# mhalushka/miRge3.0

Measured on AMD Instinct MI355X. Metric: M reads/s through full annotation cascade; per-class counts bit-exact vs ref, higher is better.
Workload: dtype u64

## Files before the change

mirge3.0_amd/csrc/kernels_join.hpp:

```cpp
#pragma once
#define MIRGE_JOIN_LDS 2048
__global__ void k_join(const int8_t* __restrict__ res_pass, const int32_t* __restrict__ res_ref,
                       const uint32_t* __restrict__ counts, uint32_t n, int32_t S, int32_t n_pass,
                       int32_t exact_pass, int32_t iso_pass, unsigned long long* __restrict__ class_sums,
                       unsigned long long* __restrict__ exact, unsigned long long* __restrict__ iso) {
    __shared__ unsigned long long acc[MIRGE_JOIN_LDS];
    const int cells = n_pass * S;
    const bool use_lds = cells <= MIRGE_JOIN_LDS;
    if (use_lds) {
        for (int c = threadIdx.x; c < cells; c += blockDim.x) acc[c] = 0ull;
        __syncthreads();
    }
    for (uint32_t i = blockIdx.x * blockDim.x + threadIdx.x; i < n; i += gridDim.x * blockDim.x) {
        const int p = res_pass[i];
        if (p < 0) continue;
        const int32_t ref = res_ref[i];
        for (int32_t s = 0; s < S; s++) {
            const unsigned long long c = counts[(size_t)i * S + s];
            if (!c) continue;
            if (use_lds) atomicAdd(&acc[p * S + s], c);
            else atomicAdd(&class_sums[p * S + s], c);
            if (p == exact_pass) atomicAdd(&exact[(size_t)ref * S + s], c);
            else if (p == iso_pass) atomicAdd(&iso[(size_t)ref * S + s], c);
        }
    }
    if (use_lds) {
        __syncthreads();
        for (int c = threadIdx.x; c < cells; c += blockDim.x)
            if (acc[c]) atomicAdd(&class_sums[c], acc[c]);
    }
}

struct JoinGroups {
    const int8_t* pass[MIRGE_NCLS];
    const int32_t* ref[MIRGE_NCLS];
    const uint32_t* counts[MIRGE_NCLS];
    uint32_t start[MIRGE_NCLS + 1];
    int32_t n_groups;
};
__global__ void k_join_multi(JoinGroups gs, int32_t S, int32_t n_pass, int32_t exact_pass, int32_t iso_pass,
                             unsigned long long* __restrict__ class_sums, unsigned long long* __restrict__ exact,
                             unsigned long long* __restrict__ iso) {
    __shared__ unsigned long long acc[MIRGE_JOIN_LDS];
    const int cells = n_pass * S;
    const bool use_lds = cells <= MIRGE_JOIN_LDS;
    if (use_lds) {
        for (int c = threadIdx.x; c < cells; c += blockDim.x) acc[c] = 0ull;
        __syncthreads();
    }
    const uint32_t total = gs.start[gs.n_groups];
    for (uint32_t t = blockIdx.x * blockDim.x + threadIdx.x; t < total; t += gridDim.x * blockDim.x) {
        int k = 0;
#pragma unroll
        for (int q = 1; q < MIRGE_NCLS; q++) if (q < gs.n_groups && t >= gs.start[q]) k = q;
        const uint32_t i = t - gs.start[k];
        const int8_t* gp = nullptr; const int32_t* gr = nullptr; const uint32_t* gc = nullptr;
#pragma unroll
        for (int q = 0; q < MIRGE_NCLS; q++) if (q == k) { gp = gs.pass[q]; gr = gs.ref[q]; gc = gs.counts[q]; }
        const int p = gp[i];
        if (p < 0) continue;
        const int32_t ref = gr[i];
        for (int32_t s = 0; s < S; s++) {
            const unsigned long long c = gc[(size_t)i * S + s];
            if (!c) continue;
            if (use_lds) atomicAdd(&acc[p * S + s], c);
            else atomicAdd(&class_sums[p * S + s], c);
            if (p == exact_pass) atomicAdd(&exact[(size_t)ref * S + s], c);
            else if (p == iso_pass) atomicAdd(&iso[(size_t)ref * S + s], c);
        }
    }
    if (use_lds) {
        __syncthreads();
        for (int c = threadIdx.x; c < cells; c += blockDim.x)
            if (acc[c]) atomicAdd(&class_sums[c], acc[c]);
    }
}

#define MIRGE_JOIN_ROWS_THREADS 1024
#define MIRGE_JOIN_ROWS_CELLS 6144
__global__ void __launch_bounds__(MIRGE_JOIN_ROWS_THREADS)
k_join_rows(JoinGroups gs, int32_t S, int32_t n_pass, int32_t exact_pass, int32_t iso_pass, uint32_t n_tab,
            unsigned long long* __restrict__ partial) {
    extern __shared__ __attribute__((aligned(16))) unsigned long long j_acc[];
    const uint32_t n_cls = (uint32_t)(n_pass * S), W = n_cls + 2 * n_tab;
    for (uint32_t c = threadIdx.x; c < W; c += blockDim.x) j_acc[c] = 0ull;
    __syncthreads();
    const uint32_t total = gs.start[gs.n_groups];
    if (gs.n_groups == 1 && S == 1) {
        const int8_t* __restrict__ gp = gs.pass[0]; const int32_t* __restrict__ gr = gs.ref[0]; const uint32_t* __restrict__ gc = gs.counts[0];
        const uint64_t stride = (uint64_t)gridDim.x * blockDim.x;
        for (uint64_t t0 = (uint64_t)blockIdx.x * blockDim.x + threadIdx.x; t0 < total; t0 += 4 * stride) {
            int p[4]; uint32_t r[4]; unsigned long long c[4];
#pragma unroll
            for (int u = 0; u < 4; u++) {
                const uint64_t i = t0 + (uint64_t)u * stride;
                const bool in = i < total;
                p[u] = in ? (int)gp[i] : -1;
                r[u] = in ? (uint32_t)gr[i] : 0u;
                c[u] = in ? (unsigned long long)gc[i] : 0ull;
            }
#pragma unroll
            for (int u = 0; u < 4; u++) {
                if (p[u] < 0 || !c[u]) continue;
                atomicAdd(&j_acc[p[u]], c[u]);
                if (p[u] == exact_pass) atomicAdd(&j_acc[n_cls + r[u]], c[u]);
                else if (p[u] == iso_pass) atomicAdd(&j_acc[n_cls + n_tab + r[u]], c[u]);
            }
        }
    } else
    for (uint32_t t = blockIdx.x * blockDim.x + threadIdx.x; t < total; t += gridDim.x * blockDim.x) {
        int k = 0;
#pragma unroll
        for (int q = 1; q < MIRGE_NCLS; q++) if (q < gs.n_groups && t >= gs.start[q]) k = q;
        const int8_t* gp = gs.pass[0]; const int32_t* gr = gs.ref[0]; const uint32_t* gc = gs.counts[0];
#pragma unroll
        for (int q = 1; q < MIRGE_NCLS; q++) if (q == k) { gp = gs.pass[q]; gr = gs.ref[q]; gc = gs.counts[q]; }
        const uint32_t i = t - gs.start[k];
        const int p = gp[i];
        if (p < 0) continue;
        const uint32_t ref = (uint32_t)gr[i];
        for (int32_t s = 0; s < S; s++) {
            const unsigned long long c = gc[(size_t)i * S + s];
            if (!c) continue;
            atomicAdd(&j_acc[p * S + s], c);
            if (p == exact_pass) atomicAdd(&j_acc[n_cls + (size_t)ref * S + s], c);
            else if (p == iso_pass) atomicAdd(&j_acc[n_cls + n_tab + (size_t)ref * S + s], c);
        }
    }
    __syncthreads();
    unsigned long long* row = partial + (size_t)blockIdx.x * W;
    for (uint32_t c = threadIdx.x; c < W; c += blockDim.x) row[c] = j_acc[c];
}
__global__ void __launch_bounds__(1024)
k_join_reduce(const unsigned long long* __restrict__ partial, uint32_t rows, uint32_t W, unsigned long long* __restrict__ tables,
              unsigned long long* __restrict__ host_out) {
    __shared__ unsigned long long s_part[16][64];
    const uint32_t lane = threadIdx.x & 63, wave = threadIdx.x >> 6;
    const uint32_t c = blockIdx.x * 64 + lane;
    unsigned long long sum = 0ull;
    if (c < W)
        for (uint32_t r = wave; r < rows; r += 16) sum += partial[(size_t)r * W + c];
    s_part[wave][lane] = sum;
    __syncthreads();
    if (wave == 0 && c < W) {
        unsigned long long tot = 0ull;
#pragma unroll
        for (int w = 0; w < 16; w++) tot += s_part[w][lane];
        if (host_out) host_out[c] = tables[c] + tot;
        else if (tot) tables[c] += tot;
    }
}

template <typename T>
__global__ void k_scatter_out(const T* __restrict__ in, uint32_t n, uint32_t base,
                              const uint32_t* __restrict__ orig, T* __restrict__ out) {
    for (uint32_t j = blockIdx.x * blockDim.x + threadIdx.x; j < n; j += gridDim.x * blockDim.x)
        out[orig ? orig[j] : base + j] = in[j];
}



#define MIRGE_TALLY_MAXPOS 32
struct TallyOut {
    unsigned long long *n_seqs, *seq_true, *count_true, *canon, *kept_exact, *census;
    int8_t *diag, *state;
};

struct TallyMember {
    const int8_t* res_pass; const int32_t* res_ref; const uint32_t* counts; int32_t S, exact_pass, iso_pass;
    const int32_t* fam_of_ref; const double* freq;
    __device__ __forceinline__ bool operator()(uint32_t i) const {
        const int p = res_pass[i];
        if (p != exact_pass && p != iso_pass) return false;
        const int32_t f = fam_of_ref[res_ref[i]];
        bool member = f >= 0 && p == exact_pass;
        if (f >= 0 && p == iso_pass)
            for (int32_t s = 0; s < S; s++) member |= (double)counts[(size_t)i * S + s] * freq[s] >= 1.0;
        return member;
    }
};
struct IsoMember {
    const int8_t* res_pass; int32_t exact_pass, iso_pass; const uint32_t* orig; uint32_t base; const int32_t* slot_of_read;
    __device__ __forceinline__ bool operator()(uint32_t i) const {
        const int p = res_pass[i];
        return (p == exact_pass || p == iso_pass) && slot_of_read[orig ? orig[i] : base + i] >= 0;
    }
};

template <class Pred, int BLOCK>
__global__ void k_member_list(uint32_t n, uint32_t chunk, Pred pred, uint32_t* __restrict__ list, uint32_t* __restrict__ n_list) {
    __shared__ uint32_t s_wave[BLOCK / 64 + 1];
    const int lane = threadIdx.x & 63, wave = threadIdx.x >> 6;
    const uint32_t lo = blockIdx.x * chunk, hi = min(n, lo + chunk);
    uint32_t run = 0;
    for (uint32_t i0 = lo; i0 < hi; i0 += BLOCK) {
        const uint32_t i = i0 + threadIdx.x;
        const bool member = i < hi && pred(i);
        const unsigned long long bal = __ballot(member);
        if (lane == 0) s_wave[wave] = (uint32_t)__popcll(bal);
        __syncthreads();
        uint32_t before = 0, tot = 0;
#pragma unroll
        for (int w = 0; w < BLOCK / 64; w++) { const uint32_t c = s_wave[w]; if (w < wave) before += c; tot += c; }
        if (member) list[lo + run + before + (uint32_t)__popcll(bal & ((1ull << lane) - 1ull))] = i;
        run += tot;
        __syncthreads();
    }
    if (threadIdx.x == 0) n_list[blockIdx.x] = run;
}

__global__ void k_tally(GroupView<1> g, uint32_t base, const uint32_t* __restrict__ orig, const int8_t* __restrict__ res_pass,
                        const int32_t* __restrict__ res_ref, const uint32_t* __restrict__ counts, int32_t S,
                        int32_t exact_pass, int32_t iso_pass, const int32_t* __restrict__ fam_of_ref,
                        const uint64_t* __restrict__ tgt_bits, const uint8_t* __restrict__ tgt_len,
                        const uint8_t* __restrict__ retained, const double* __restrict__ freq, TallyOut o,
                        const uint32_t* __restrict__ list, const uint32_t* __restrict__ n_list, uint32_t chunk) {
    const uint32_t n_members = n_list[blockIdx.x];
    for (uint32_t k = threadIdx.x; k < n_members; k += blockDim.x) {
        const uint32_t i = list[(size_t)blockIdx.x * chunk + k];
        const int p = res_pass[i];
        const uint32_t h = orig ? orig[i] : base + i;
        const int32_t f = fam_of_ref[res_ref[i]];
        const uint64_t tw = tgt_bits[f];
        const int Lt = tgt_len[f], Lr = g.len[i];
        const uint64_t rw = g.seq[i];
        const uint64_t rn = g.nmask ? g.nmask[i] : 0ull;
        int best = 0, best_i = 0, best_j = 0, d = 0;
        const int nd = Lr + Lt - 1;
        for (int k = 0; k < nd + 3; k++) {
            const int dd = k < 3 ? k - 1 : k - 3 - (Lr - 1);
            if (dd <= -Lr || dd >= Lt) continue;
            const int i0 = dd > 0 ? dd : 0, i1 = min(Lt, dd + Lr), j0 = i0 - dd;
            if (2 * (i1 - i0) < best) continue;
            const uint64_t x = (tw >> (2 * i0)) ^ (rw >> (2 * j0));
            uint64_t m2 = ((x | (x >> 1)) & 0x5555555555555555ull) | ((rn >> (2 * j0)) & 0x5555555555555555ull);
            m2 = (m2 | (m2 >> 1)) & 0x3333333333333333ull;
            m2 = (m2 | (m2 >> 2)) & 0x0F0F0F0F0F0F0F0Full;
            m2 = (m2 | (m2 >> 4)) & 0x00FF00FF00FF00FFull;
            m2 = (m2 | (m2 >> 8)) & 0x0000FFFF0000FFFFull;
            const uint32_t mis = (uint32_t)(m2 | (m2 >> 16));
            int run = 0;
            for (int t = 0; t < i1 - i0; t++) {
                run = max(0, run + (((mis >> t) & 1u) ? -1 : 2));
                const int ti = i0 + t, rj = j0 + t;
                if (run > best || (run == best && run > 0 && (ti < best_i || (ti == best_i && rj < best_j)))) {
                    best = run; best_i = ti; best_j = rj; d = dd;
                }
            }
        }
        bool state = d <= 1;
        if (state) {
            const int hd_t = d < 0 ? -d : 0, hd_s = d > 0 ? d : 0;
            const int A = max(hd_t + Lt, hd_s + Lr);
            const int last = min(A - hd_t - 1 - 3, hd_s + Lr - 1);
            int mism = 0, match = 0;
            for (int pos = hd_t; pos <= last; pos++) {
                const int rj = pos - hd_s, q = pos - hd_t;
                if (rj < 0) continue;
                const bool eq = q < Lt && !((rn >> (2 * rj)) & 1ull) && (((tw >> (2 * q)) & 3ull) == ((rw >> (2 * rj)) & 3ull));
                if (eq) match++; else mism++;
            }
            state = !(mism > 1 || match < Lt - 3 - 1 - (d == 1 ? 1 : 0));
        }
        o.diag[h] = (int8_t)d;
        o.state[h] = state ? 1 : 0;
        const bool keep = state && (!retained || retained[h]);
        bool sub = false;
        if (keep && rn == 0ull && Lr <= Lt) {
            const uint64_t m = mirge_lowmask2(Lr);
            for (int a = 0; a + Lr <= Lt && !sub; a++) sub = ((tw >> (2 * a)) & m) == rw;
        }
        for (int32_t s = 0; s < S; s++) {
            const unsigned long long c = counts[(size_t)i * S + s];
            if (!c) continue;
            const size_t fs = (size_t)f * S + s;
            atomicAdd(&o.n_seqs[fs], 1ull);
            if (keep) {
                atomicAdd(&o.seq_true[fs], 1ull);
                atomicAdd(&o.count_true[fs], c);
                if (sub) atomicAdd(&o.canon[fs], c);
                if (p == exact_pass) atomicAdd(&o.kept_exact[fs], 1ull);
            }
            for (int q = max(0, d); q < Lt - 5 && q - d < Lr; q++) {
                const int rj = q - d;
                if ((rn >> (2 * rj)) & 1ull) continue;
                const int cb = (int)((tw >> (2 * q)) & 3ull), rb = (int)((rw >> (2 * rj)) & 3ull);
                if (cb == rb) continue;
                unsigned long long* cell = &o.census[((((size_t)f * MIRGE_TALLY_MAXPOS + q) * 16 + cb * 4 + rb) * 3) * S + s];
                atomicAdd(cell, c);
                if (state) atomicAdd(cell + S, c);
                if (keep) atomicAdd(cell + 2 * S, c);
            }
        }
    }
}
```

mirge3.0_amd/csrc/native_cascade.hpp:

```cpp
#pragma once
struct ResGroup {
    uint32_t n = 0;
    int8_t* pass = nullptr;
    uint32_t* pos = nullptr;
    int8_t* mm = nullptr;
    int32_t* ref = nullptr;
    int32_t* off = nullptr;
};
struct mirge_result {
    mirge_ctx* ctx = nullptr;
    int64_t n = 0;
    int32_t n_pass = 0;
    ResGroup g[MIRGE_NGROUPS];
    const mirge_reads* reads = nullptr;
    uint32_t n_refs[MIRGE_MAX_PASSES] = {0};
    uint32_t* dmeta = nullptr;
};

extern "C" void mirge_result_destroy(mirge_result* r) {
    if (!r) return;
    (void)join_pending_now(r->ctx);
    for (auto& g : r->g) {
        r->ctx->release(g.pass); r->ctx->release(g.pos); r->ctx->release(g.mm);
        r->ctx->release(g.ref); r->ctx->release(g.off);
    }
    r->ctx->release(r->dmeta);
    delete r;
}

static int merged_library(mirge_ctx* c, const mirge_lib* const* members, int n, mirge_lib** out) {
    std::vector<uint64_t> uids;
    for (int i = 0; i < n; i++) uids.push_back(members[i]->uid);
    for (auto& m : c->merged)
        if (m.uids == uids) { *out = m.lib; return 0; }
    std::string seq;
    std::vector<int64_t> off;
    std::vector<const MirgeHostLib*> hl;
    for (int i = 0; i < n; i++) hl.push_back(&members[i]->h);
    merged_library_text(hl.data(), n, seq, off);
    mirge_lib* L = nullptr;
    CHECK(mirge_lib_create(c, seq.data(), off.data(), (int64_t)off.size() - 1, &L));
    c->merged.push_back(mirge_ctx::Merged{uids, L});
    *out = L;
    return 0;
}

static int prepare_tables(mirge_lib* lib, const mirge_policy& pol, const int32_t* hist, bool long_present) {
    MirgePolicy p;
    std::memcpy(&p, &pol, sizeof(p));
    std::vector<ShapeJob> wanted;
    std::vector<bool> seen(MIRGE_SHAPE_SLOTS, false);
    for (int L = 1; L <= MIRGE_MAX_READ_LEN + 1; L++) {
        const bool lng = L > MIRGE_MAX_READ_LEN;
        if (lng ? !long_present : !hist[L]) continue;
        if (p.len_lt > 0 && !(L < p.len_lt) && !(lng && p.len_lt > MIRGE_MAX_READ_LEN + 1)) continue;
        if (p.len_gt > 0 && !(L > p.len_gt) && !lng) continue;
        int lo = L, hi = L;
        if (lng) lo = hi = 31 + p.trim5 + p.trim3;
        if (p.ttail) { lo = 1; hi = (lng ? 31 + p.trim5 + p.trim3 : L - 3); }
        for (int l0 = lo; l0 <= hi; l0++) {
            const int l = l0 - p.trim5 - p.trim3;
            if (l < 1 || l <= p.mm) continue;
            const int np = mirge_probe_count(p, l, lib->kmax, lib->h.total);
            for (int q = 0; q < np; q++) {
                MirgeProbe pr;
                mirge_probe_at(p, l, lib->kmax, lib->h.total, q, pr);
                if (pr.k1 <= 0) continue;
                const int sid = mirge_shape_id(pr.k1, pr.gap, pr.k2);
                if (seen[sid]) continue;
                seen[sid] = true;
                wanted.emplace_back();
                wanted.back().k1 = pr.k1; wanted.back().gap = pr.gap; wanted.back().k2 = pr.k2;
            }
        }
    }
    return lib_prepare_shapes(lib, wanted);
}

static uint32_t* heavy_counters(mirge_ctx* c, const char* gtag) {
    if (!c->casc_big_t || !c->heavy_cnt) return nullptr;
    for (int gi = 0; gi < MIRGE_NGROUPS; gi++)
        if (std::strcmp(group_tag(gi), gtag) == 0) return c->heavy_cnt + 2 * gi;
    return c->heavy_cnt;
}
template <int W>
static void launch_heavy(mirge_ctx* c, const ReadGroup& rg, const ResGroup& out, const FusedSteps* dsteps, const ResolveTable& rt, const char* gtag,
                         uint32_t* hcnt, const uint32_t* hlist, const GroupView<W>& v, bool with_resolve) {
    char name[40];
    std::snprintf(name, sizeof(name), "k_cascade_heavy%s", gtag);
    LaunchScope ls(c, name, 0.0);
    const uint32_t grid = (uint32_t)c->n_cu * 2u;
    int32_t* rr = with_resolve ? out.ref : nullptr;
    int32_t* ro = with_resolve ? out.off : nullptr;
    if (rg.nmask)
        hipLaunchKernelGGL((k_cascade_heavy<W, true>), dim3(grid), dim3(MIRGE_HEAVY_THREADS), 0, c->cur, dsteps, rt, v, hcnt, hlist, out.pass, out.pos, out.mm, rr, ro);
    else
        hipLaunchKernelGGL((k_cascade_heavy<W, false>), dim3(grid), dim3(MIRGE_HEAVY_THREADS), 0, c->cur, dsteps, rt, v, hcnt, hlist, out.pass, out.pos, out.mm, rr, ro);
}

template <int W>
static int cascade_group(mirge_ctx* c, const ReadGroup& rg, ResGroup& out, const std::vector<PassStep>& steps,
                         const mirge_policy* pol, const ResolveTable& rt, const char* gtag,
                         const uint32_t* n_dev = nullptr, uint32_t n_cap = 0, const BulkWalks* dwalks = nullptr) {
    out.n = n_dev ? 0 : rg.n;
    if (!n_dev && !rg.n) return 0;
    const uint32_t n = n_dev ? n_cap : rg.n;
    CHECK(dalloc(c, &out.pass, n));
    CHECK(dalloc(c, &out.pos, n));
    CHECK(dalloc(c, &out.mm, n));
    CHECK(dalloc(c, &out.ref, n));
    CHECK(dalloc(c, &out.off, n));
    static int wg_per_cu[9] = {0};
    if (!wg_per_cu[W]) {
        int nb = 0;
        hipFuncAttributes fa;
        HIPOK(hipOccupancyMaxActiveBlocksPerMultiprocessor(&nb, reinterpret_cast<const void*>(k_cascade_bulk<W, false, true>), MIRGE_BLOCK, 0));
        HIPOK(hipFuncGetAttributes(&fa, reinterpret_cast<const void*>(k_cascade_bulk<W, false, true>)));
        const int by_regs = 512 / std::max(16, (fa.numRegs + 15) / 16 * 16);
        wg_per_cu[W] = std::max(1, std::min({nb, by_regs, W == 1 ? MIRGE_BULK_WAVES : 6}));
        if (std::getenv("MIRGE_WG_PER_CU")) wg_per_cu[W] = std::max(1, std::atoi(std::getenv("MIRGE_WG_PER_CU")));
        if (std::getenv("MIRGE_HOST_TIMING"))
            std::fprintf(stderr, "[host] k_pass<%d>: %d VGPRs, occupancy query %d -> %d workgroups per CU\n", W, fa.numRegs, nb, wg_per_cu[W]);
    }
    const uint32_t grid = (uint32_t)std::min<size_t>((size_t)grid_for(c, n), (size_t)c->n_cu * wg_per_cu[W]);
    uint32_t cap = (n + grid - 1) / grid;
    cap = (cap + MIRGE_BLOCK - 1) / MIRGE_BLOCK * MIRGE_BLOCK;
    uint32_t *actA = nullptr, *actB = nullptr, *seg_n = nullptr;
    uint32_t* const hcnt = heavy_counters(c, gtag);
    uint32_t* hlist = nullptr;
    if (hcnt) CHECK(dalloc(c, &hlist, (size_t)n));
    CHECK(dalloc(c, &actA, (size_t)grid * cap));
    CHECK(dalloc(c, &actB, (size_t)grid * cap));
    CHECK(dalloc(c, &seg_n, (size_t)grid * (MIRGE_MAX_PASSES + 3)));
    if (steps.empty()) {
        HIPOK(hipMemsetAsync(out.pass, 0xFF, n, c->cur));
        HIPOK(hipMemsetAsync(out.mm, 0xFF, n, c->cur));
    }
    GroupView<W> v = view_of<W>(rg);
    if (n_dev) v.n = n;
    const uint32_t* act_in = nullptr;
    uint32_t* act_out = actA;
    int stage = 0;
    char name[32];
    std::vector<std::pair<int, int>> stage_of_pass;
    static const bool bulk_fused = !(std::getenv("MIRGE_BULK_FUSED") && std::atoi(std::getenv("MIRGE_BULK_FUSED")) == 0);
    if (bulk_fused && dwalks && steps.size() > 1) {
        std::snprintf(name, sizeof(name), "k_cascade_bulk%s", gtag);
        LaunchScope ls(c, name, 0.0);
        if (ls.rec >= 0)
            for (size_t k = 0; k < steps.size(); k++) stage_of_pass.emplace_back(ls.rec, (int)k);
#define MIRGE_LAUNCH_BULK(HASN_, REP_)                                                                                                              \
    hipLaunchKernelGGL((k_cascade_bulk<W, HASN_, REP_>), dim3(grid), dim3(MIRGE_BLOCK), 0, c->cur, dwalks, v, actA, actB, seg_n, cap, out.pass, out.pos, \
                       out.mm, n_dev, hcnt, hlist)
        if (rg.nmask) { if (c->casc_rep) MIRGE_LAUNCH_BULK(true, true); else MIRGE_LAUNCH_BULK(true, false); }
        else { if (c->casc_rep) MIRGE_LAUNCH_BULK(false, true); else MIRGE_LAUNCH_BULK(false, false); }
#undef MIRGE_LAUNCH_BULK
        stage = (int)steps.size();
        if (c->profiling && W == 1) {
            if (c->wg_pinned_words < 2 * (size_t)grid) {
                if (c->wg_pinned) (void)hipHostFree(c->wg_pinned);
                c->wg_pinned = nullptr; c->wg_pinned_words = 0;
                if (hipHostMalloc((void**)&c->wg_pinned, 2 * (size_t)grid * 4, hipHostMallocDefault) == hipSuccess) c->wg_pinned_words = 2 * (size_t)grid;
            }
            if (c->wg_pinned_words >= 2 * (size_t)grid) {
                HIPOK(hipMemcpyAsync(c->wg_pinned, seg_n + (size_t)grid * (MIRGE_MAX_PASSES + 1), 2 * (size_t)grid * 4, hipMemcpyDeviceToHost, c->cur));
                c->wg_grid = grid;
            }
        }
    } else
    for (const PassStep& st : steps) {
        const int32_t p = st.p0;
        MirgePolicy mp;
        std::memcpy(&mp, &pol[p], sizeof(mp));
        mp.reserved = hcnt ? (int32_t)c->casc_big_t : 0;
        {
            if (st.np > 1) std::snprintf(name, sizeof(name), "k_pass[%d-%d]%s", (int)p, (int)(p + st.np - 1), gtag);
            else std::snprintf(name, sizeof(name), "k_pass[%d]%s", (int)p, gtag);
            LaunchScope ls(c, name, 0.0);
            if (ls.rec >= 0) stage_of_pass.emplace_back(ls.rec, stage);
            const uint32_t* sn_in = seg_n + (size_t)grid * (stage > 0 ? stage - 1 : 0);
            uint32_t* sn_out = seg_n + (size_t)grid * stage;
#define MIRGE_LAUNCH_PASS(SLOT)                                                                                       \
    hipLaunchKernelGGL((k_pass<W, SLOT>), dim3(grid), dim3(MIRGE_BLOCK), 0, c->cur, st.lib->view(), mp, st.mi, st.dplan, v, act_in, \
                       sn_in, act_out, sn_out, cap, p, out.pass, out.pos, out.mm, n_dev, hcnt, hlist)
            switch (p) {
                case 0: MIRGE_LAUNCH_PASS(0); break;
                case 1: MIRGE_LAUNCH_PASS(1); break;
                case 2: MIRGE_LAUNCH_PASS(2); break;
                case 3: MIRGE_LAUNCH_PASS(3); break;
                case 4: MIRGE_LAUNCH_PASS(4); break;
                case 5: MIRGE_LAUNCH_PASS(5); break;
                case 6: MIRGE_LAUNCH_PASS(6); break;
                case 7: MIRGE_LAUNCH_PASS(7); break;
                case 8: MIRGE_LAUNCH_PASS(8); break;
                case 9: MIRGE_LAUNCH_PASS(9); break;
                default: MIRGE_LAUNCH_PASS(15); break;
            }
#undef MIRGE_LAUNCH_PASS
        }
        act_in = act_out;
        act_out = (act_out == actA) ? actB : actA;
        stage++;
    }
    if (hcnt && stage > 0) launch_heavy<W>(c, rg, out, c->casc_dsteps, rt, gtag, hcnt, hlist, v, false);
    {
        std::snprintf(name, sizeof(name), "k_resolve%s", gtag);
        LaunchScope ls(c, name, n);
        hipLaunchKernelGGL(k_resolve, dim3(grid_for(c, n)), dim3(MIRGE_BLOCK), 0, c->cur, rt, out.pass, out.pos, n, out.ref, out.off, n_dev);
    }
    if (c->profiling && c->prof_units && stage > 0 && !stage_of_pass.empty()) {
        const size_t words = (size_t)grid * stage;
        if (c->prof_used + words <= MIRGE_PROF_PINNED_WORDS) {
            uint32_t* dst = c->prof_pinned + c->prof_used;
            HIPOK(hipMemcpyAsync(dst, seg_n, words * 4, hipMemcpyDeviceToHost, c->cur));
            for (auto& sp : stage_of_pass) c->prof_pending.push_back(ProfUnits{sp.first, sp.second, grid, dst, (double)n});
            c->prof_used += words;
        }
    }
    c->defer(actA); c->defer(actB); c->defer(seg_n); c->defer(hlist);
    return 0;
}

template <int W>
static int cascade_group_fused(mirge_ctx* c, const ReadGroup& rg, ResGroup& out, const FusedSteps* dsteps,
                               const ResolveTable& rt, const char* gtag) {
    out.n = rg.n;
    if (!rg.n) return 0;
    const uint32_t n = rg.n;
    CHECK(dalloc(c, &out.pass, n));
    CHECK(dalloc(c, &out.pos, n));
    CHECK(dalloc(c, &out.mm, n));
    CHECK(dalloc(c, &out.ref, n));
    CHECK(dalloc(c, &out.off, n));
    uint32_t* const hcnt = heavy_counters(c, gtag);
    uint32_t* hlist = nullptr;
    if (hcnt) CHECK(dalloc(c, &hlist, (size_t)n));
    char name[32];
    static const uint32_t spec_max = std::getenv("MIRGE_SPEC_MAX") ? (uint32_t)std::strtoul(std::getenv("MIRGE_SPEC_MAX"), nullptr, 10) : 32768u;
    const int nsteps = (int)c->casc_steps.size();
    if (n <= spec_max && nsteps > 1) {
        unsigned long long* answers = nullptr;
        const uint32_t rounds = (n + MIRGE_BLOCK - 1) / MIRGE_BLOCK, stride = rounds * MIRGE_BLOCK;
        CHECK(dalloc(c, &answers, (size_t)nsteps * stride));
        const dim3 grid(rounds, (unsigned)nsteps);
        {
            std::snprintf(name, sizeof(name), "k_cascade_spec%s", gtag);
            LaunchScope ls(c, name, n);
#define MIRGE_LAUNCH_SPEC(HASN_, REP_)                                                                                                          \
    hipLaunchKernelGGL((k_cascade_spec<W, HASN_, REP_>), grid, dim3(MIRGE_BLOCK), 0, c->cur, dsteps, view_of<W>(rg), answers, stride)
            if (rg.nmask) { if (c->casc_rep) MIRGE_LAUNCH_SPEC(true, true); else MIRGE_LAUNCH_SPEC(true, false); }
            else { if (c->casc_rep) MIRGE_LAUNCH_SPEC(false, true); else MIRGE_LAUNCH_SPEC(false, false); }
#undef MIRGE_LAUNCH_SPEC
            hipLaunchKernelGGL(k_cascade_pick<W>, dim3(rounds), dim3(MIRGE_BLOCK), 0, c->cur, dsteps, rt, n, stride,
                               (const unsigned long long*)answers, out.pass, out.pos, out.mm, out.ref, out.off, hcnt, hlist);
        }
        if (hcnt) launch_heavy<W>(c, rg, out, dsteps, rt, gtag, hcnt, hlist, view_of<W>(rg), true);
        c->defer(hlist); c->defer(answers);
        return 0;
    }
    std::snprintf(name, sizeof(name), "k_cascade_fused%s", gtag);
    {
        LaunchScope ls(c, name, n);
        const uint32_t grid = std::min<uint32_t>((n + MIRGE_BLOCK - 1) / MIRGE_BLOCK, (uint32_t)c->n_cu * 8);
#define MIRGE_LAUNCH_FUSED(HASN_, REP_)                                                                                                        \
    hipLaunchKernelGGL((k_cascade_fused<W, HASN_, REP_>), dim3(grid), dim3(MIRGE_BLOCK), 0, c->cur, dsteps, rt, view_of<W>(rg), out.pass, out.pos, \
                       out.mm, out.ref, out.off, hcnt, hlist)
        if (rg.nmask) { if (c->casc_rep) MIRGE_LAUNCH_FUSED(true, true); else MIRGE_LAUNCH_FUSED(true, false); }
        else { if (c->casc_rep) MIRGE_LAUNCH_FUSED(false, true); else MIRGE_LAUNCH_FUSED(false, false); }
#undef MIRGE_LAUNCH_FUSED
    }
    if (hcnt) launch_heavy<W>(c, rg, out, dsteps, rt, gtag, hcnt, hlist, view_of<W>(rg), true);
    c->defer(hlist);
    return 0;
}

static int cascade_group_long(mirge_ctx* c, const ReadGroup& rg, ResGroup& out, const FusedSteps* dsteps, const ResolveTable& rt,
                              const char* gtag) {
    out.n = rg.n;
    if (!rg.n) return 0;
    const uint32_t n = rg.n;
    CHECK(dalloc(c, &out.pass, n));
    CHECK(dalloc(c, &out.pos, n));
    CHECK(dalloc(c, &out.mm, n));
    CHECK(dalloc(c, &out.ref, n));
    CHECK(dalloc(c, &out.off, n));
    char name[32];
    std::snprintf(name, sizeof(name), "k_cascade_long%s", gtag);
    LaunchScope ls(c, name, n);
    const uint32_t grid = std::min<uint32_t>((n + 63) / 64, (uint32_t)c->n_cu * 8);
    hipLaunchKernelGGL(k_cascade_long, dim3(grid), dim3(64), 0, c->cur, dsteps, rt, long_view_of(rg), out.pass, out.pos, out.mm, out.ref, out.off);
    return 0;
}

static int cascade_prepare(mirge_ctx* c, const mirge_lib* const* libs, const mirge_policy* pol, int32_t n_pass,
                           const int32_t* hist, bool long_present, std::vector<PassStep>& steps, ResolveTable& rt, const FusedSteps** dsteps_out,
                           const BulkWalks** dwalks_out) {
    for (int p = 0; p < MIRGE_MAX_PASSES; p++) { rt.ref_start[p] = nullptr; rt.coarse[p] = nullptr; rt.n_refs[p] = 0; }
    steps.clear();
    for (int32_t p = 0; p < n_pass; p++) {
        if (!libs[p]) continue;
        if (libs[p]->ctx->device != c->device) return fail(-1, "library lives on another device");
        if (pol[p].mm < 0 || pol[p].mm > 3 || pol[p].trim5 < 0 || pol[p].trim5 > 31 || pol[p].trim3 < 0)
            return fail(-1, "unsupported policy");
        rt.ref_start[p] = libs[p]->dref_start;
        rt.coarse[p] = libs[p]->dcoarse;
        rt.n_refs[p] = (uint32_t)libs[p]->n_refs;
    }
    for (int32_t p = 0; p < n_pass;) {
        if (!libs[p]) { p++; continue; }
        int np = 1;
        uint64_t total = libs[p]->h.total;
        static const bool merge_on = !(std::getenv("MIRGE_MERGE_PASSES") && std::getenv("MIRGE_MERGE_PASSES")[0] == '0');
        while (merge_on && np < 4 && p + np < n_pass && libs[p + np] && std::memcmp(&pol[p + np], &pol[p], sizeof(mirge_policy)) == 0 &&
               total + libs[p + np]->h.total < 0xFFFFFFF0ull) {
            bool distinct = true;
            for (int q = 0; q < np; q++) distinct &= libs[p + q] != libs[p + np];
            if (!distinct) break;
            total += libs[p + np]->h.total;
            np++;
        }
        PassStep st;
        st.p0 = p; st.np = np;
        st.mi.n = np;
        for (int i = 0; i < 4; i++) st.mi.bound[i] = 0;
        if (np == 1) st.lib = libs[p];
        else {
            mirge_lib* m = nullptr;
            CHECK(merged_library(c, libs + p, np, &m));
            st.lib = m;
            uint64_t b = 0;
            for (int i = 0; i < np; i++) { st.mi.bound[i] = (uint32_t)b; b += libs[p + i]->h.total; }
        }
        CHECK(prepare_tables(const_cast<mirge_lib*>(st.lib), pol[p], hist, long_present));
        steps.push_back(st);
        p += np;
    }
    for (auto& st : steps) {
        MirgePolicy mp;
        std::memcpy(&mp, &pol[st.p0], sizeof(mp));
        const MirgePlanTable* dp = nullptr;
        for (auto& e : c->plans)
            if (e.uid == st.lib->uid && std::memcmp(&e.pol, &mp, sizeof(mp)) == 0) { dp = e.dplan; break; }
        if (!dp) {
            auto h = std::make_unique<MirgePlanTable>();
            mirge_plan_table_fill(mp, st.lib->kmax, st.lib->h.total, *h);
            MirgePlanTable* d = nullptr;
            HIPOK(hipMalloc((void**)&d, sizeof(MirgePlanTable)));
            HIPOK(hipMemcpy(d, h.get(), sizeof(MirgePlanTable), hipMemcpyHostToDevice));
            c->plans.push_back(mirge_ctx::PlanEntry{st.lib->uid, mp, d});
            dp = d;
        }
        st.dplan = dp;
    }
    static const uint32_t big_t_env = std::getenv("MIRGE_BIG_T") ? (uint32_t)std::strtoul(std::getenv("MIRGE_BIG_T"), nullptr, 10) : 8192u;
    static const bool big_t_forced = std::getenv("MIRGE_BIG_T") != nullptr;
    static const int rep_env = std::getenv("MIRGE_CASCADE_REP") ? std::atoi(std::getenv("MIRGE_CASCADE_REP")) : -1;
    c->casc_big_t = big_t_forced ? big_t_env : 0;
    c->casc_rep = rep_env > 0 || big_t_forced;
    for (auto& st : steps) {
        if (st.lib->max_bucket > 0 && rep_env != 0) c->casc_rep = true;
        if (big_t_env && st.lib->max_bucket > big_t_env) c->casc_big_t = big_t_env;
    }
    if (!c->casc_rep) c->casc_big_t = 0;
    if (c->casc_big_t && !c->heavy_cnt) {
        HIPOK(hipMalloc((void**)&c->heavy_cnt, 2 * MIRGE_NGROUPS * 4));
        HIPOK(hipMemset(c->heavy_cnt, 0, 2 * MIRGE_NGROUPS * 4));
    }
    auto fs = std::make_unique<FusedSteps>();
    std::memset(fs.get(), 0, sizeof(FusedSteps));
    fs->n = (int32_t)steps.size();
    for (size_t i = 0; i < steps.size(); i++) {
        FusedStep& f = fs->s[i];
        f.lib = steps[i].lib->view();
        std::memcpy(&f.pol, &pol[steps[i].p0], sizeof(MirgePolicy));
        f.pol.reserved = (int32_t)c->casc_big_t;
        f.mi = steps[i].mi;
        f.plan = steps[i].dplan;
        f.pass_id = steps[i].p0;
    }
    const FusedSteps* dsteps = nullptr;
    const FusedSteps* fs_host = fs.get();
    for (auto& e : c->fused)
        if (std::memcmp(e.host.get(), fs.get(), sizeof(FusedSteps)) == 0) { dsteps = e.dev; break; }
    if (!dsteps) {
        if (c->fused.size() >= 64) {
            HIPOK(hipDeviceSynchronize());
            for (auto& e : c->fused) (void)hipFree(e.dev);
            c->fused.clear();
        }
        FusedSteps* d = nullptr;
        HIPOK(hipMalloc((void**)&d, sizeof(FusedSteps)));
        HIPOK(hipMemcpy(d, fs.get(), sizeof(FusedSteps), hipMemcpyHostToDevice));
        c->fused.push_back(mirge_ctx::FusedEntry{std::move(fs), d});
        dsteps = d;
    }
    *dsteps_out = dsteps;
    static const bool exact_on = !(std::getenv("MIRGE_EXACT_WALKS") && std::atoi(std::getenv("MIRGE_EXACT_WALKS")) == 0);
    std::vector<ExactStep> ex(steps.size());
    std::vector<char> is_exact(steps.size(), 0);
    {
        bool dropped = false;
        for (size_t i = 0; i < steps.size() && exact_on; i++)
            if (steps[i].lib->ctx == c) dropped |= lib_exact_trim(const_cast<mirge_lib*>(steps[i].lib));
        if (dropped) {
            for (auto& e : c->walks) (void)hipFree(e.dev);
            c->walks.clear();
        }
    }
    for (size_t i = 0; i < steps.size() && exact_on; i++) {
        const PassStep& st = steps[i];
        MirgePolicy p;
        std::memcpy(&p, &pol[st.p0], sizeof(p));
        if (st.np != 1 || p.mm != 0 || st.lib->ctx != c) continue;
        uint32_t lmask = 0;
        int lmax = 0;
        for (int L = 1; L <= 31; L++) {
            if (!hist[L]) continue;
            if (p.len_lt > 0 && !(L < p.len_lt)) continue;
            if (p.len_gt > 0 && !(L > p.len_gt)) continue;
            const int lo = p.ttail ? 1 : L, hi = p.ttail ? L - 3 : L;
            for (int l0 = lo; l0 <= hi; l0++) {
                const int l = l0 - p.trim5 - p.trim3;
                if (l < 1 || l <= p.mm) continue;
                lmask |= 1u << l;
                lmax = std::max(lmax, l);
            }
        }
        if (p.mode == 0 && lmax > p.seedlen) continue;
        mirge_lib::ExactTab tab;
        CHECK(lib_exact_table(const_cast<mirge_lib*>(st.lib), lmask, &tab));
        if (!tab.slots) continue;
        ExactStep& e = ex[i];
        e.slots = tab.slots; e.T = st.lib->dT; e.mask = tab.mask; e.pass_id = st.p0; e.step = (int32_t)i; e.pol = p;
        is_exact[i] = 1;
    }
    if (c->walks.size() + 2 > 64) {
        HIPOK(hipDeviceSynchronize());
        for (auto& e : c->walks) (void)hipFree(e.dev);
        c->walks.clear();
    }
    for (int wide = 0; wide < 2; wide++) {
        auto bw = std::make_unique<BulkWalks>();
        std::memset(bw.get(), 0, sizeof(BulkWalks));
        for (size_t i = 0; i < steps.size();) {
            BulkWalk& w = bw->w[bw->n++];
            if (!wide && is_exact[i]) w.pre = ex[i++];
            if (!wide && !MIRGE_EXACT_RIDE && w.pre.slots) {
                if (i < steps.size() && is_exact[i]) w.post = ex[i++];
                continue;
            }
            if (i < steps.size() && (wide || !is_exact[i])) {
                w.has_main = 1;
                w.main_step = (int32_t)i;
                w.main = fs_host->s[i];
                i++;
                const MirgePolicy& mp = w.main.pol;
                if (!wide && i < steps.size() && is_exact[i] && !mp.trim5 && !mp.trim3 && !mp.ttail) w.post = ex[i++];
            }
        }
        const BulkWalks* dwalks = nullptr;
        for (auto& e : c->walks)
            if (std::memcmp(e.host.get(), bw.get(), sizeof(BulkWalks)) == 0) { dwalks = e.dev; break; }
        if (!dwalks) {
            BulkWalks* d = nullptr;
            HIPOK(hipMalloc((void**)&d, sizeof(BulkWalks)));
            HIPOK(hipMemcpy(d, bw.get(), sizeof(BulkWalks), hipMemcpyHostToDevice));
            c->walks.push_back(mirge_ctx::WalksEntry{std::move(bw), d});
            dwalks = d;
        }
        dwalks_out[wide] = dwalks;
    }
    return 0;
}

static int cascade_config(mirge_ctx* c, const mirge_lib* const* libs, const mirge_policy* pol, int32_t n_pass, const int32_t* hist,
                          bool long_present) {
    std::string key;
    key.append(reinterpret_cast<const char*>(&n_pass), sizeof(n_pass));
    for (int32_t p = 0; p < n_pass; p++) {
        const uint64_t uid = libs[p] ? libs[p]->uid : 0;
        key.append(reinterpret_cast<const char*>(&uid), sizeof(uid));
        key.append(reinterpret_cast<const char*>(&pol[p]), sizeof(mirge_policy));
    }
    for (int L = 0; L <= MIRGE_MAX_READ_LEN; L++) key.push_back(hist[L] ? 1 : 0);
    key.push_back(long_present ? 1 : 0);
    if (c->casc_key != key) {
        c->casc_key.clear();
        CHECK(cascade_prepare(c, libs, pol, n_pass, hist, long_present, c->casc_steps, c->casc_rt, &c->casc_dsteps, c->casc_dwalks));
        c->casc_key = key;
    }
    return 0;
}

static int cascade_launch_groups(mirge_ctx* c, const mirge_reads* R, mirge_result* res, const mirge_policy* pol, int skip, int big_is = -1) {
    const std::vector<PassStep>& steps = c->casc_steps;
    const ResolveTable& rt = c->casc_rt;
    const FusedSteps* dsteps = c->casc_dsteps;
    const uint32_t fused_max = small_fused_max();
    int rc = 0;
    const int big = big_is >= 0 ? big_is : largest_group(R);
    CHECK(stream_fork(c));
    int order[MIRGE_NGROUPS], no = 0;
    for (int gi = 0; gi < MIRGE_NGROUPS; gi++) if (gi != big) order[no++] = gi;
    std::stable_sort(order, order + no, [&](int a, int b) { return R->g[a].n > R->g[b].n; });
    order[no++] = big;
    uint32_t n[MIRGE_NGROUPS];
    int slot[MIRGE_NGROUPS];
    for (int gi = 0; gi < MIRGE_NGROUPS; gi++) n[gi] = R->g[gi].n;
    if (small_group_slots(n, big, skip, slot) && !c->xaux_forked) CHECK(xaux_fork(c));
    for (int k = 0; k < MIRGE_NGROUPS && rc == 0; k++) {
        const int gi = order[k];
        if (gi == skip) continue;
        c->cur = gi == big ? c->stream : c->aux;
        if (is_long_group(gi)) {
            rc = cascade_group_long(c, R->g[gi], res->g[gi], dsteps, rt, group_tag(gi));
            continue;
        }
        if (gi != big && R->g[gi].n <= fused_max) {
            if (slot[gi] >= 0) c->cur = c->xaux[slot[gi]];
            MIRGE_BY_WIDTH(gi, rc, cascade_group_fused<W>(c, R->g[gi], res->g[gi], dsteps, rt, group_tag(gi)));
            continue;
        }
        MIRGE_BY_WIDTH(gi, rc, cascade_group<W>(c, R->g[gi], res->g[gi], steps, pol, rt, group_tag(gi), nullptr, 0, c->casc_dwalks[W == 1 ? 0 : 1]));
    }
    c->x0_gathered = false;
    if (rc == 0 && c->xaux_forked && c->xaux_used) {
        hipError_t e = hipSuccess;
        for (int k = 1; k < MIRGE_N_SLOTS && e == hipSuccess; k++) {
            e = hipEventRecord(c->ev_xjoin[k], c->xaux[k]);
            if (e == hipSuccess) e = hipStreamWaitEvent(c->xaux[0], c->ev_xjoin[k], 0);
        }
        c->x0_gathered = e == hipSuccess;
    }
    c->cur = c->stream;
    if (rc == 0) c->join_pending = true;
    else { int jr = stream_join(c); (void)jr; }
    return rc;
}

static void reads_lengths_present(const mirge_reads* R, int32_t* hist) {
    if (R->hist_valid) { std::memcpy(hist, R->len_hist, sizeof(int32_t) * (MIRGE_MAX_READ_LEN + 1)); return; }
    std::memset(hist, 0, sizeof(int32_t) * (MIRGE_MAX_READ_LEN + 1));
    for (int gi = 0; gi < MIRGE_NGROUPS; gi++) {
        const ReadGroup& g = R->g[gi];
        if (!g.n || is_long_group(gi)) continue;
        const int w = kGroupW[gi];
        int lo = w == 1 ? 1 : (w == 2 ? 32 : (w == 4 ? 65 : 129)), hi = w == 1 ? 31 : (w == 2 ? 64 : (w == 4 ? 128 : MIRGE_MAX_READ_LEN));
        for (int L = lo; L <= hi; L++) hist[L] = 1;
    }
}

extern "C" int mirge_cascade_run(mirge_ctx* c, const mirge_reads* R, const mirge_lib* const* libs,
                                 const mirge_policy* pol, int32_t n_pass, mirge_result** out) {
    HostClock hc("cascade");
    if (!c || !R || !libs || !pol || !out || n_pass < 1 || n_pass > MIRGE_MAX_PASSES)
        return fail(-1, "mirge_cascade_run: bad argument");
    HIPOK(hipSetDevice(c->device)); CHECK(join_pending_now(c));
    int32_t hist[MIRGE_MAX_READ_LEN + 1];
    reads_lengths_present(R, hist);
    CHECK(cascade_config(c, libs, pol, n_pass, hist, R->long_max > 0));
    hc.lap("plans+fused");
    auto res = std::make_unique<mirge_result>();
    res->ctx = c; res->n = R->n; res->n_pass = n_pass; res->reads = R;
    for (int32_t p = 0; p < n_pass; p++) res->n_refs[p] = libs[p] ? (uint32_t)libs[p]->n_refs : 0u;
    const int rc = cascade_launch_groups(c, R, res.get(), pol, -1);
    hc.lap("enqueue+join");
    if (rc) { mirge_result_destroy(res.release()); return rc; }
    *out = res.release();
    return 0;
}

extern "C" int mirge_cascade_prepare(mirge_ctx* c, const mirge_reads* R, const mirge_lib* const* libs, const mirge_policy* pol,
                                     int32_t n_pass) {
    if (!c || !R || !libs || !pol || n_pass < 1 || n_pass > MIRGE_MAX_PASSES) return fail(-1, "mirge_cascade_prepare: bad argument");
    HIPOK(hipSetDevice(c->device)); CHECK(join_pending_now(c));
    int32_t hist[MIRGE_MAX_READ_LEN + 1];
    reads_lengths_present(R, hist);
    CHECK(cascade_config(c, libs, pol, n_pass, hist, R->long_max > 0));
    HIPOK(hipStreamSynchronize(c->stream));
    return 0;
}

extern "C" int mirge_cascade_wg_times(mirge_ctx* c, uint32_t* ticks_out, int32_t cap, int32_t* grid_out, int32_t* khz_out) {
    if (!c || !grid_out) return fail(-1, "mirge_cascade_wg_times: bad argument");
    CHECK(mirge_ctx_sync(c));
    *grid_out = (int32_t)c->wg_grid;
    int khz = 100000;
    (void)hipDeviceGetAttribute(&khz, hipDeviceAttributeWallClockRate, c->device);
    if (khz_out) *khz_out = khz;
    for (uint32_t b = 0; ticks_out && b < c->wg_grid && (int32_t)b < cap; b++) ticks_out[b] = c->wg_pinned[c->wg_grid + b] - c->wg_pinned[b];
    return 0;
}

extern "C" int mirge_cascade_walks(mirge_ctx* c, int32_t* walks) {
    if (!c || !walks) return fail(-1, "mirge_cascade_walks: bad argument");
    walks[0] = walks[1] = walks[2] = 0;
    for (auto& e : c->walks) {
        if (e.dev != c->casc_dwalks[0]) continue;
        walks[0] = e.host->n;
        for (int i = 0; i < e.host->n; i++) {
            const BulkWalk& w = e.host->w[i];
            walks[1] += (w.pre.slots != nullptr) + (w.post.slots != nullptr);
            walks[2] += (w.pre.slots != nullptr) + (w.post.slots != nullptr) + (w.has_main != 0);
        }
    }
    return 0;
}

extern "C" int mirge_collapse_cascade(mirge_ctx* c, const mirge_reads* raw, const mirge_lib* const* libs, const mirge_policy* pol,
                                      int32_t n_pass, mirge_reads** uniq, int64_t* n_uniq, mirge_result** out) {
    if (!c || !raw || !libs || !pol || !uniq || !out || n_pass < 1 || n_pass > MIRGE_MAX_PASSES)
        return fail(-1, "mirge_collapse_cascade: bad argument");
    HIPOK(hipSetDevice(c->device)); CHECK(join_pending_now(c));
    mirge_reads* U = nullptr;
    if (!raw->hist_valid || raw->n == 0) {
        CHECK(mirge_collapse(c, raw, nullptr, 1, &U, n_uniq));
        const int rc = mirge_cascade_run(c, U, libs, pol, n_pass, out);
        if (rc) { mirge_reads_destroy(U); return rc; }
        *uniq = U;
        return 0;
    }
    CHECK(cascade_config(c, libs, pol, n_pass, raw->len_hist, raw->long_max > 0));
    auto res = std::make_unique<mirge_result>();
    res->ctx = c; res->n_pass = n_pass;
    for (int32_t p = 0; p < n_pass; p++) res->n_refs[p] = libs[p] ? (uint32_t)libs[p]->n_refs : 0u;
    const size_t prof_mark = c->prof_pending.size();
    int hooked_group = -1;
    CollapseHook hook;
    hook.pre_sync = [&](mirge_reads* partial, const CollapseTmp*, uint32_t* dmeta, int big) -> int {
        ReadGroup rg = partial->g[big];
        rg.n = raw->g[big].n;
        c->cur = c->stream;
        const int rc = cascade_group<1>(c, rg, res->g[big], c->casc_steps, pol, c->casc_rt, group_tag(big), dmeta + big, raw->g[big].n, c->casc_dwalks[0]);
        if (rc == 0) { hooked_group = big; c->overlap_mode = true; }
        return rc;
    };
    hook.small_ready = [&](mirge_reads* partial, int big) -> int {
        return cascade_launch_groups(c, partial, res.get(), pol, big, big);
    };
    hook.discard = [&]() {
        (void)hipStreamSynchronize(c->stream);
        (void)hipStreamSynchronize(c->aux);
        for (int k = 0; k < MIRGE_N_XAUX; k++) (void)hipStreamSynchronize(c->xaux[k]);
        c->overlap_mode = false;
        c->join_pending = false;
        c->xaux_used = false;
        c->x0_gathered = c->aux_drained = false;
        for (int gi = 0; gi < MIRGE_NGROUPS; gi++) {
            if (gi != hooked_group && !res->g[gi].pass) continue;
            ResGroup& g = res->g[gi];
            c->release(g.pass); c->release(g.pos); c->release(g.mm); c->release(g.ref); c->release(g.off);
            g = ResGroup();
        }
        hooked_group = -1;
        c->prof_pending.resize(std::min(c->prof_pending.size(), prof_mark));
        c->flush_deferred();
    };
    int rc = collapse_impl(c, raw, nullptr, 1, &U, n_uniq, &hook);
    if (rc) { c->overlap_mode = false; mirge_result_destroy(res.release()); return rc; }
    if (!hook.ran) {
        res.reset();
        rc = mirge_cascade_run(c, U, libs, pol, n_pass, out);
        if (rc) { mirge_reads_destroy(U); return rc; }
        *uniq = U;
        return 0;
    }
    res->n = U->n; res->reads = U; res->dmeta = hook.dmeta;
    res->g[hooked_group].n = U->g[hooked_group].n;
    for (size_t i = prof_mark; i < c->prof_pending.size(); i++) c->prof_pending[i].n_first = (double)U->g[hooked_group].n;
    if (!hook.small_ran) rc = cascade_launch_groups(c, U, res.get(), pol, hooked_group);
    c->overlap_mode = false;
    if (rc) { (void)hipStreamSynchronize(c->stream); mirge_result_destroy(res.release()); mirge_reads_destroy(U); return rc; }
    *uniq = U;
    *out = res.release();
    return 0;
}

template <typename T>
static int fetch_field(mirge_ctx* c, const mirge_result* res, T* host_out, T* ResGroup::*field) {
    if (!host_out || !res->n) return 0;
    T* dfull = nullptr;
    CHECK(dalloc(c, &dfull, (size_t)res->n));
    for (int gi = 0; gi < MIRGE_NGROUPS; gi++) {
        const ResGroup& g = res->g[gi];
        const ReadGroup& rg = res->reads->g[gi];
        if (!g.n) continue;
        hipLaunchKernelGGL(k_scatter_out<T>, dim3(grid_for(c, g.n)), dim3(MIRGE_BLOCK), 0, c->stream,
                           (const T*)(g.*field), g.n, rg.base, (const uint32_t*)rg.orig, dfull);
    }
    HIPOK(hipMemcpyAsync(host_out, dfull, (size_t)res->n * sizeof(T), hipMemcpyDeviceToHost, c->stream));
    HIPOK(hipStreamSynchronize(c->stream));
    c->release(dfull);
    return 0;
}

extern "C" int mirge_result_fetch(mirge_ctx* c, const mirge_result* res, int8_t* pass_out, int32_t* ref_out,
                                  int32_t* off_out, int8_t* mm_out) {
    if (!c || !res) return fail(-1, "mirge_result_fetch: bad argument");
    HIPOK(hipSetDevice(c->device)); CHECK(join_pending_now(c));
    CHECK(fetch_field<int8_t>(c, res, pass_out, &ResGroup::pass));
    CHECK(fetch_field<int32_t>(c, res, ref_out, &ResGroup::ref));
    CHECK(fetch_field<int32_t>(c, res, off_out, &ResGroup::off));
    CHECK(fetch_field<int8_t>(c, res, mm_out, &ResGroup::mm));
    return 0;
}
```

mirge3.0_amd/csrc/native_collapse.hpp:

```cpp
#pragma once
struct CollapseTmp {
    uint32_t *rep = nullptr, *firstj = nullptr, *cnt = nullptr, *slot_of = nullptr, *blocksum = nullptr;
    KeySlot* slots = nullptr;
    uint8_t* flag = nullptr;
    const uint32_t* cnt_base = nullptr;
    uint32_t cnt_stride = 1, nb = 0;
    bool partitioned = false;
    uint4 *rec1 = nullptr, *rec2 = nullptr;
    uint32_t *cnt1 = nullptr, *cnt2 = nullptr, *off2 = nullptr, *hist = nullptr;
    uint32_t *shard_cur = nullptr, shard_cap = 0, *s_cnt = nullptr, *s_first = nullptr, rec_thresh = 0;
    uint64_t* s_seq = nullptr;
    uint8_t* s_len = nullptr;
    uint32_t G = 0, B = 0, NB1 = 0, NB2 = 1, W2 = 1, RPW = 0, cap1 = 0, shift2 = 0, cap = MIRGE_PART_CAP;
    uint64_t slab = 0;
};
#ifndef MIRGE_PART_CACHE
#define MIRGE_PART_CACHE 4096
#endif
#ifndef MIRGE_PART_RETRY_BYTES
#define MIRGE_PART_RETRY_BYTES (64ull << 30)
#endif
#define MIRGE_META_OVERFLOW 10
#define MIRGE_META_LONG_BASES 12
#define MIRGE_META_HIST 16
#define MIRGE_META_RECORDS (((MIRGE_META_HIST + MIRGE_MAX_READ_LEN + 1 + 63) & ~63) + 64)
#define MIRGE_META_WORDS (MIRGE_META_RECORDS + 64)

static const char* group_tag(int gi) {
    static const char* t[MIRGE_NGROUPS] = {".w1", ".w2", ".w4", ".w8", ".wl", ".w1n", ".w2n", ".w4n", ".w8n", ".wln"};
    return t[gi];
}

static uint32_t part_region_cap(double mean) {
    const double c = 1.25 * mean + 8.0 * std::sqrt(mean) + 64.0;
    return ((uint32_t)c + 3u) & ~3u;
}

static void part_len_hist(mirge_ctx* c, const ReadGroup& out, const CollapseTmp& t, uint32_t* dmeta, int gi) {
    if (!t.partitioned || !out.len) return;
    hipStream_t const was = c->cur;
    c->cur = c->aux;
    {
        LaunchScope ls(c, "k_len_hist", 0.0);
        hipLaunchKernelGGL(k_len_hist, dim3((unsigned)c->n_cu * 2), dim3(256), 0, c->aux, (const uint8_t*)out.len, (const uint32_t*)(dmeta + gi),
                           dmeta + MIRGE_META_HIST);
    }
    c->cur = was;
}

static int collapse_part_rest(mirge_ctx* c, int gi, const ReadGroup& in, ReadGroup& out, CollapseTmp& t, uint32_t* dmeta, int part = 0) {
    const bool two = t.NB2 > 1;
    if (part != 2 && two) {
        LaunchScope ls(c, "k_part_split.w1", in.n);
        hipLaunchKernelGGL(k_part_split, dim3(t.NB1 * t.W2), dim3(MIRGE_PART_THREADS), (MIRGE_PART_MAXREG + t.NB2) * 4, c->cur,
                           t.rec1, t.cnt1, t.hist, t.G, t.B, t.cap1, t.W2, t.RPW, t.shift2, t.NB2, t.slab, t.rec2, t.off2, t.cnt2);
    }
    if (part != 1) {
        LaunchScope ls(c, "k_part_dedup.w1", in.n);
        const uint4* rec = two ? t.rec2 : t.rec1;
        const uint32_t* cnt = two ? t.cnt2 : t.cnt1;
        const uint32_t* off = two ? t.off2 : nullptr;
        const uint32_t R = two ? t.W2 : t.G;
        const uint64_t rcap = two ? t.slab : (uint64_t)t.cap1;
        const bool sh = t.shard_cur != nullptr;
        uint64_t* const oseq = reinterpret_cast<uint64_t*>(out.seq);
        uint8_t* const olen = reinterpret_cast<uint8_t*>(out.len);
        if (t.cap == 2048)
            hipLaunchKernelGGL(k_part_dedup<2048>, dim3(t.B), dim3(MIRGE_DEDUP_THREADS), 2048 * 16 + 4096, c->cur, rec, cnt, off, R, rcap, t.NB2,
                               oseq, olen, out.counts, out.first, dmeta + gi, (uint32_t*)nullptr, dmeta + MIRGE_META_OVERFLOW, t.shard_cur, t.shard_cap,
                               (const uint32_t*)(dmeta + MIRGE_META_RECORDS), t.rec_thresh, t.s_seq, t.s_len, t.s_cnt, t.s_first);
        else
            hipLaunchKernelGGL(k_part_dedup<MIRGE_PART_CAP>, dim3(t.B), dim3(MIRGE_DEDUP_THREADS), MIRGE_PART_CAP * 16 + 4096, c->cur, rec,
                               cnt, off, R, rcap, t.NB2, oseq, olen, out.counts, out.first, dmeta + gi, (uint32_t*)nullptr,
                               dmeta + MIRGE_META_OVERFLOW, t.shard_cur, t.shard_cap, (const uint32_t*)(dmeta + MIRGE_META_RECORDS), t.rec_thresh,
                               t.s_seq, t.s_len, t.s_cnt, t.s_first);
        if (sh) {
            LaunchScope ls2(c, "k_part_compact.w1", in.n);
            hipLaunchKernelGGL(k_part_compact, dim3((unsigned)c->n_cu * 8), dim3(256), 0, c->cur, (const uint32_t*)t.shard_cur, t.shard_cap,
                               (const uint64_t*)t.s_seq, (const uint8_t*)t.s_len, (const uint32_t*)t.s_cnt, (const uint32_t*)t.s_first,
                               oseq, olen, out.counts, out.first, dmeta + gi, (const uint32_t*)(dmeta + MIRGE_META_RECORDS), t.rec_thresh);
        }
    }
    return 0;
}

template <int W>
static int collapse_phase_a(mirge_ctx* c, int gi, const ReadGroup& in, ReadGroup& out, CollapseTmp& t,
                            const int32_t* dsample, int32_t S, uint32_t* dmeta, int attempt, int stage = 0,
                            const uint32_t* dweight = nullptr) {
    const bool force_atomic = attempt >= 2 || (attempt == 1 && (uint64_t)in.n * 2048ull > MIRGE_PART_RETRY_BYTES);
    if (!in.n) return 0;
    if (stage == 2 && t.partitioned) return collapse_part_rest(c, gi, in, out, t, dmeta, 2);
    const bool key_path = (W == 1) && !in.nmask && S == 1 && !dweight;
    const uint64_t need = key_path ? (uint64_t)in.n + in.n / 2 : 2ull * in.n;
    uint64_t tsize64 = 1024;
    while (tsize64 < need) tsize64 <<= 1;
    if (tsize64 > (1ull << 31)) return fail(-5, "collapse: a read group of " + std::to_string(in.n) + " reads needs a hash table beyond 2^31 slots");
    const uint32_t tsize = (uint32_t)tsize64;
    const uint32_t per_block = MIRGE_BLOCK * MIRGE_SCAN_ITEMS;
    t.nb = (in.n + per_block - 1) / per_block;
    GroupView<W> v = view_of<W>(in);
    char name[48];
    const uint32_t* first_base;
    uint32_t first_stride;
    if (key_path && !force_atomic && in.n >= 65536) {
        t.partitioned = true;
        uint32_t B = 64;
        static const bool small_part = std::getenv("MIRGE_TEST_SMALL_PART") != nullptr;
        while (!small_part && B < 32768 && (uint64_t)B * 2048 < in.n) B <<= 1;
        t.cap = (!small_part && (uint64_t)B * MIRGE_PART_SMALL >= in.n) ? 2048u : (uint32_t)MIRGE_PART_CAP;
        static const uint32_t nb1_env = std::getenv("MIRGE_PART_NB1") ? (uint32_t)std::max(1, std::min(256, std::atoi(std::getenv("MIRGE_PART_NB1")))) : 0u;
        const uint32_t nb1_cap = nb1_env ? nb1_env : B >= 32768 ? 256u : B >= 16384 ? 128u : (uint32_t)MIRGE_PART_B1;
        const uint32_t NB1 = std::min<uint32_t>(B, nb1_cap), NB2 = B / NB1;
        const uint32_t CS = B > 16384 ? 1024 : MIRGE_PART_CACHE;
        const int agg_lds = (int)(CS * 16 + NB1 * 4 + (NB2 > 1 ? B * 4 : 0) + 64);
        static std::mutex attr_mu;
        static std::vector<int> attr_done;
        {
            std::lock_guard<std::mutex> lk(attr_mu);
            if (std::find(attr_done.begin(), attr_done.end(), c->device) == attr_done.end()) {
                HIPOK(hipFuncSetAttribute(reinterpret_cast<const void*>(k_part_agg), hipFuncAttributeMaxDynamicSharedMemorySize,
                                          1024 * 16 + 256 * 4 + 32768 * 4 + 64));
                HIPOK(hipFuncSetAttribute(reinterpret_cast<const void*>(k_part_dedup<MIRGE_PART_CAP>),
                                          hipFuncAttributeMaxDynamicSharedMemorySize, MIRGE_PART_CAP * 16 + 4096));
                attr_done.push_back(c->device);
            }
        }
        int lg = 0; while ((1u << lg) < B) lg++;
        int lg1 = 0; while ((1u << lg1) < NB1) lg1++;
        const uint32_t G = std::min<uint32_t>(256, (in.n + 2047) / 2048);
        uint32_t chunk = (in.n + G - 1) / G;
        chunk = (chunk + MIRGE_BLOCK - 1) / MIRGE_BLOCK * MIRGE_BLOCK;
        const uint32_t shift1 = 64 - lg1, shift2 = 64 - lg;
        const uint32_t w2_want = std::max<uint32_t>(1, (uint32_t)MIRGE_PART_W2 * (uint32_t)MIRGE_PART_B1 / NB1);
        const uint32_t W2 = NB2 > 1 ? std::min<uint32_t>(w2_want, G) : 1, RPW = (G + W2 - 1) / W2;
        static const bool small_region = std::getenv("MIRGE_TEST_SMALL_REGION") != nullptr;
        const uint32_t cap1 = attempt == 1 ? chunk
                                           : small_region ? std::max<uint32_t>(4, chunk / NB1 / 2 & ~3u) : part_region_cap((double)chunk / NB1);
        const uint64_t slab = (uint64_t)RPW * cap1;
        static const bool part_oom = std::getenv("MIRGE_TEST_PART_OOM") != nullptr;
        if (part_oom && attempt == 1) return fail(-3, "hipMalloc: out of memory (MIRGE_TEST_PART_OOM)");
        CHECK(dalloc(c, &t.rec1, (size_t)NB1 * G * cap1));
        CHECK(dalloc(c, &t.cnt1, (size_t)NB1 * G));
        static const int sharded_env = std::getenv("MIRGE_DEDUP_SHARDED") ? std::atoi(std::getenv("MIRGE_DEDUP_SHARDED")) : -1;
        static const double rec_share = std::getenv("MIRGE_DEDUP_REC_SHARE") ? std::atof(std::getenv("MIRGE_DEDUP_REC_SHARE")) : 0.45;
        const bool sharded = sharded_env != 0;
        t.rec_thresh = sharded_env > 0 ? 0xFFFFFFFFu : (uint32_t)std::min<double>(4.0e9, rec_share * (double)in.n);
        if (sharded && attempt == 0 && !small_part) {
            t.shard_cap = in.n / MIRGE_DEDUP_SHARDS + in.n / (8 * MIRGE_DEDUP_SHARDS) + 65536u;
            const size_t sn = (size_t)t.shard_cap * MIRGE_DEDUP_SHARDS;
            CHECK(dalloc(c, &t.shard_cur, (size_t)MIRGE_DEDUP_SHARDS * MIRGE_DEDUP_SHARD_STRIDE));
            CHECK(dalloc(c, &t.s_seq, sn));
            CHECK(dalloc(c, &t.s_len, sn));
            CHECK(dalloc(c, &t.s_cnt, sn));
            CHECK(dalloc(c, &t.s_first, sn));
        }
        if (NB2 > 1) {
            CHECK(dalloc(c, &t.hist, (size_t)G * B));
            CHECK(dalloc(c, &t.rec2, (size_t)NB1 * W2 * slab));
            CHECK(dalloc(c, &t.cnt2, (size_t)B * W2));
            CHECK(dalloc(c, &t.off2, (size_t)B * W2));
        }
        out.W = 1;
        CHECK(dalloc(c, &out.seq, (size_t)in.n));
        CHECK(dalloc(c, &out.len, (size_t)in.n));
        CHECK(dalloc(c, &out.counts, (size_t)in.n));
        CHECK(dalloc(c, &out.first, (size_t)in.n));
        GroupView<1> v1 = view_of<1>(in);
        {
            LaunchScope ls(c, "k_part_agg.w1", in.n);
            hipLaunchKernelGGL(k_part_agg, dim3(G), dim3(MIRGE_PART_THREADS), agg_lds, c->cur, v1, in.orig, in.base, chunk, shift1, NB1,
                               shift2, B, CS, cap1, t.rec1, t.cnt1, t.hist, dmeta + MIRGE_META_OVERFLOW, dmeta + MIRGE_META_RECORDS, t.shard_cur);
        }
        t.G = G; t.B = B; t.NB1 = NB1; t.NB2 = NB2; t.W2 = W2; t.RPW = RPW; t.cap1 = cap1; t.slab = slab; t.shift2 = shift2;
        if (stage == 1) return collapse_part_rest(c, gi, in, out, t, dmeta, 1);
        return collapse_part_rest(c, gi, in, out, t, dmeta);
    }
    if (stage == 1) return 0;
    CHECK(dalloc(c, &t.slot_of, in.n));
    CHECK(dalloc(c, &t.flag, (size_t)t.nb * per_block));
    CHECK(dalloc(c, &t.blocksum, t.nb));
    if (key_path) {
        CHECK(dalloc(c, &t.slots, tsize));
        HIPOK(hipMemsetAsync(t.slots, 0, (size_t)tsize * sizeof(KeySlot), c->cur));
        LaunchScope ls(c, "k_collapse_insert_key.w1", in.n);
        hipLaunchKernelGGL(k_collapse_insert_key, dim3(grid_for(c, in.n)), dim3(MIRGE_BLOCK), 0, c->cur,
                           view_of<1>(in), t.slots, t.slot_of, tsize - 1);
        first_base = reinterpret_cast<const uint32_t*>(t.slots) + 2; first_stride = 4;
        t.cnt_base = reinterpret_cast<const uint32_t*>(t.slots) + 3; t.cnt_stride = 4;
    } else {
        CHECK(dalloc(c, &t.rep, tsize));
        CHECK(dalloc(c, &t.firstj, tsize));
        CHECK(dalloc(c, &t.cnt, (size_t)tsize * S));
        hipLaunchKernelGGL(k_collapse_init, dim3(grid_for(c, (size_t)tsize * S)), dim3(MIRGE_BLOCK), 0, c->cur, t.rep, t.firstj, t.cnt,
                           tsize, (uint64_t)tsize * (uint64_t)S);
        std::snprintf(name, sizeof(name), "k_collapse_insert%s", group_tag(gi));
        LaunchScope ls(c, name, in.n);
        static const int ins_per_cu = std::getenv("MIRGE_INSERT_WG_PER_CU") ? std::max(1, std::atoi(std::getenv("MIRGE_INSERT_WG_PER_CU"))) : 0;
        const int ins_grid = std::min(grid_for(c, in.n), c->n_cu * (ins_per_cu ? ins_per_cu : (in.n < (2u << 20) ? 8 : 2)));
        const uint32_t seed = std::min<uint32_t>(in.n, MIRGE_COLLAPSE_SEED);
        hipLaunchKernelGGL(k_collapse_insert<W>, dim3((seed + MIRGE_BLOCK - 1) / MIRGE_BLOCK), dim3(MIRGE_BLOCK), 0, c->cur,
                           v, t.rep, t.firstj, t.cnt, t.slot_of, tsize - 1, dsample, in.orig, in.base, S, 0u, seed, dweight);
        if (in.n > seed)
            hipLaunchKernelGGL(k_collapse_insert<W>, dim3(ins_grid), dim3(MIRGE_BLOCK), 0, c->cur,
                               v, t.rep, t.firstj, t.cnt, t.slot_of, tsize - 1, dsample, in.orig, in.base, S, seed, in.n, dweight);
        first_base = t.firstj; first_stride = 1;
        t.cnt_base = t.cnt; t.cnt_stride = (uint32_t)S;
    }
    {
        std::snprintf(name, sizeof(name), "k_heads_blocksum%s", group_tag(gi));
        LaunchScope ls(c, name, in.n);
        hipLaunchKernelGGL(k_heads_blocksum, dim3(t.nb), dim3(MIRGE_BLOCK), 0, c->cur, t.slot_of, first_base, first_stride,
                           key_path ? 1u : 0u, in.n, in.len, t.flag, t.blocksum, dmeta + MIRGE_META_HIST);
    }
    {
        LaunchScope ls(c, "k_scan_blocksums", t.nb);
        hipLaunchKernelGGL(k_scan_blocksums, dim3(1), dim3(MIRGE_BLOCK), 0, c->cur, t.blocksum, t.nb, dmeta + gi);
    }
    return 0;
}

template <int W>
static int collapse_phase_b(mirge_ctx* c, int gi, const ReadGroup& in, ReadGroup& out, CollapseTmp& t, int32_t S,
                            uint32_t U, uint32_t out_base, const uint32_t* dmeta) {
    out.W = W; out.n = U; out.base = out_base;
    if (in.n && !t.partitioned) {
        CHECK(dalloc(c, &out.seq, (size_t)W * U));
        CHECK(dalloc(c, &out.len, (size_t)U));
        if (in.nmask) CHECK(dalloc(c, &out.nmask, (size_t)W * U));
        CHECK(dalloc(c, &out.counts, (size_t)U * S));
        CHECK(dalloc(c, &out.first, (size_t)U));
        char name[48];
        std::snprintf(name, sizeof(name), "k_collapse_scatter%s", group_tag(gi));
        LaunchScope ls(c, name, in.n);
        hipLaunchKernelGGL(k_collapse_scatter<W>, dim3(t.nb), dim3(MIRGE_BLOCK), 0, c->cur, view_of<W>(in), t.slot_of,
                           t.flag, t.cnt_base, t.cnt_stride, t.blocksum, dmeta + gi, in.orig, in.base, S, out.seq,
                           out.len, out.nmask, out.counts, out.first);
    }
    return 0;
}

static int collapse_phase_a_long(mirge_ctx* c, int gi, const ReadGroup& in, CollapseTmp& t, const int32_t* dsample, int32_t S,
                                 uint32_t* dmeta, int stage, const uint32_t* dweight) {
    if (!in.n || stage == 1) return 0;
    uint64_t tsize64 = 1024;
    while (tsize64 < 2ull * in.n) tsize64 <<= 1;
    if (tsize64 > (1ull << 31)) return fail(-5, "collapse: a read group of " + std::to_string(in.n) + " reads needs a hash table beyond 2^31 slots");
    const uint32_t tsize = (uint32_t)tsize64;
    const uint32_t per_block = MIRGE_BLOCK * MIRGE_SCAN_ITEMS;
    t.nb = (in.n + per_block - 1) / per_block;
    CHECK(dalloc(c, &t.slot_of, in.n));
    CHECK(dalloc(c, &t.flag, (size_t)t.nb * per_block));
    CHECK(dalloc(c, &t.blocksum, t.nb));
    CHECK(dalloc(c, &t.rep, tsize));
    CHECK(dalloc(c, &t.firstj, tsize));
    CHECK(dalloc(c, &t.cnt, (size_t)tsize * S));
    hipLaunchKernelGGL(k_collapse_init, dim3(grid_for(c, (size_t)tsize * S)), dim3(MIRGE_BLOCK), 0, c->cur, t.rep, t.firstj, t.cnt,
                       tsize, (uint64_t)tsize * (uint64_t)S);
    const LongView v = long_view_of(in);
    char name[48];
    {
        std::snprintf(name, sizeof(name), "k_collapse_insert%s", group_tag(gi));
        LaunchScope ls(c, name, in.n);
        hipLaunchKernelGGL(k_collapse_insert_long, dim3(grid_for(c, in.n)), dim3(MIRGE_BLOCK), 0, c->cur, v, t.rep, t.firstj, t.cnt, t.slot_of,
                           tsize - 1, dsample, in.orig, in.base, S, dweight);
    }
    t.cnt_base = t.cnt; t.cnt_stride = (uint32_t)S;
    {
        std::snprintf(name, sizeof(name), "k_heads_blocksum%s", group_tag(gi));
        LaunchScope ls(c, name, in.n);
        hipLaunchKernelGGL(k_heads_blocksum, dim3(t.nb), dim3(MIRGE_BLOCK), 0, c->cur, t.slot_of, (const uint32_t*)t.firstj, 1u, 0u, in.n,
                           (const uint8_t*)nullptr, t.flag, t.blocksum, dmeta + MIRGE_META_HIST);
        hipLaunchKernelGGL(k_long_heads_bases, dim3(grid_for(c, in.n)), dim3(MIRGE_BLOCK), 0, c->cur, t.slot_of, (const uint32_t*)t.firstj, v.len, in.n,
                           reinterpret_cast<unsigned long long*>(dmeta + MIRGE_META_LONG_BASES));
    }
    {
        LaunchScope ls(c, "k_scan_blocksums", t.nb);
        hipLaunchKernelGGL(k_scan_blocksums, dim3(1), dim3(MIRGE_BLOCK), 0, c->cur, t.blocksum, t.nb, dmeta + gi);
    }
    return 0;
}

static int collapse_phase_b_long(mirge_ctx* c, int gi, const ReadGroup& in, ReadGroup& out, CollapseTmp& t, int32_t S, uint32_t U,
                                 uint32_t out_base, const uint32_t* dmeta) {
    out.W = in.W; out.n = U; out.base = out_base;
    if (!in.n) return 0;
    CHECK(dalloc(c, &out.seq, (size_t)out.W * U));
    CHECK(dalloc(c, &out.len, (size_t)U * 2));
    if (in.nmask) CHECK(dalloc(c, &out.nmask, (size_t)out.W * U));
    CHECK(dalloc(c, &out.counts, (size_t)U * S));
    CHECK(dalloc(c, &out.first, (size_t)U));
    char name[48];
    std::snprintf(name, sizeof(name), "k_collapse_scatter%s", group_tag(gi));
    LaunchScope ls(c, name, in.n);
    hipLaunchKernelGGL(k_collapse_scatter_long, dim3(t.nb), dim3(MIRGE_BLOCK), 0, c->cur, long_view_of(in), t.slot_of, t.flag, t.cnt_base,
                       t.cnt_stride, t.blocksum, dmeta + gi, in.orig, in.base, S, out.seq, reinterpret_cast<uint16_t*>(out.len), out.nmask,
                       out.counts, out.first);
    return 0;
}

static void collapse_tmp_release(mirge_ctx* c, CollapseTmp& t) {
    c->defer(t.rep); c->defer(t.firstj); c->defer(t.cnt); c->defer(t.slots); c->defer(t.slot_of);
    c->defer(t.flag); c->defer(t.blocksum);
    c->defer(t.rec1); c->defer(t.cnt1); c->defer(t.rec2); c->defer(t.cnt2); c->defer(t.off2); c->defer(t.hist);
    c->defer(t.shard_cur); c->defer(t.s_seq); c->defer(t.s_len); c->defer(t.s_cnt); c->defer(t.s_first);
    t = CollapseTmp();
}

struct CollapseHook {
    std::function<int(mirge_reads* partial, const CollapseTmp* tmp, uint32_t* dmeta, int big)> pre_sync;
    std::function<int(mirge_reads* partial, int big)> small_ready;
    std::function<void()> discard;
    bool ran = false;
    bool small_ran = false;
    uint32_t* dmeta = nullptr;
};

static int collapse_impl(mirge_ctx* c, const mirge_reads* raw, const int32_t* sample_ids, int32_t S, mirge_reads** uniq,
                         int64_t* n_uniq, CollapseHook* hook, const uint32_t* weights = nullptr, int32_t* dsample_in = nullptr,
                         uint32_t* dweight_in = nullptr);

static uint32_t small_fused_max() {
    static const uint32_t v = std::getenv("MIRGE_FUSED_MAX") ? (uint32_t)std::strtoul(std::getenv("MIRGE_FUSED_MAX"), nullptr, 10) : (1u << 19);
    return v;
}
static bool small_group_slots(const uint32_t* n, int big, int skip, int* slot) {
    const uint32_t fused_max = small_fused_max();
    int order[MIRGE_NGROUPS], no = 0;
    for (int gi = 0; gi < MIRGE_NGROUPS; gi++) { slot[gi] = -1; if (gi != big && gi != skip) order[no++] = gi; }
    std::stable_sort(order, order + no, [&](int a, int b) { return n[a] > n[b]; });
    int n_small = 0;
    for (int k = 0; k < no; k++) if (n[order[k]] && n[order[k]] <= fused_max) n_small++;
    if (n_small <= 1) return false;
    int next = 0;
    for (int k = 0; k < no; k++) {
        const int gi = order[k];
        if (is_long_group(gi) || !n[gi] || n[gi] > fused_max) continue;
        slot[gi] = next++ % MIRGE_N_SLOTS;
    }
    return true;
}

extern "C" int mirge_collapse(mirge_ctx* c, const mirge_reads* raw, const int32_t* sample_ids, int32_t S,
                              mirge_reads** uniq, int64_t* n_uniq) {
    return collapse_impl(c, raw, sample_ids, S, uniq, n_uniq, nullptr);
}
extern "C" int mirge_collapse_weighted(mirge_ctx* c, const mirge_reads* raw, const int32_t* sample_ids, int32_t S,
                                       const uint32_t* weights, mirge_reads** uniq, int64_t* n_uniq) {
    return collapse_impl(c, raw, sample_ids, S, uniq, n_uniq, nullptr, weights);
}

static int collapse_impl(mirge_ctx* c, const mirge_reads* raw, const int32_t* sample_ids, int32_t S, mirge_reads** uniq,
                         int64_t* n_uniq, CollapseHook* hook, const uint32_t* weights, int32_t* dsample_in, uint32_t* dweight_in) {
    HostClock hc("collapse");
    if (!c || !raw || !uniq || S < 1 || (S > 1 && !sample_ids && !dsample_in)) return fail(-1, "mirge_collapse: bad argument");
    HIPOK(hipSetDevice(c->device)); CHECK(join_pending_now(c));
    int32_t* dsample = dsample_in;
    if (!dsample_in && sample_ids && raw->n) {
        for (int64_t i = 0; i < raw->n; i++)
            if (sample_ids[i] < 0 || sample_ids[i] >= S) return fail(-1, "sample id out of range");
        CHECK(dalloc(c, &dsample, (size_t)raw->n));
        HIPOK(hipMemcpyAsync(dsample, sample_ids, (size_t)raw->n * 4, hipMemcpyHostToDevice, c->stream));
    }
    uint32_t* dweight = dweight_in;
    if (!dweight_in && weights && raw->n) {
        CHECK(dalloc(c, &dweight, (size_t)raw->n));
        HIPOK(hipMemcpyAsync(dweight, weights, (size_t)raw->n * 4, hipMemcpyHostToDevice, c->stream));
    }
    auto R = std::make_unique<mirge_reads>();
    R->ctx = c; R->n_samples = S;
    uint32_t* dmeta = nullptr;
    CHECK(dalloc(c, &dmeta, MIRGE_META_WORDS));
    CollapseTmp tmp[MIRGE_NGROUPS];
    int rc = 0;
    const int big = largest_group(raw);
    bool small_done = false;
    for (int attempt = 0; attempt < 3 && rc == 0; attempt++) {
        hipError_t e0 = hipMemsetAsync(dmeta, 0, MIRGE_META_WORDS * 4, c->stream);
        if (e0 != hipSuccess) { rc = fail(-2, std::string("mirge_collapse: ") + hipGetErrorString(e0)); break; }
        rc = stream_fork(c);
        for (int k = -1; k <= MIRGE_NGROUPS && rc == 0; k++) {
            const int gi = (k < 0 || k == MIRGE_NGROUPS) ? big : k;
            if (k >= 0 && k < MIRGE_NGROUPS && gi == big) continue;
            const int stage = k < 0 ? 1 : (k == MIRGE_NGROUPS ? 2 : 0);
            c->cur = gi == big ? c->stream : c->aux;
            if (is_long_group(gi)) rc = collapse_phase_a_long(c, gi, raw->g[gi], tmp[gi], dsample, S, dmeta, stage, dweight);
            else MIRGE_BY_WIDTH(gi, rc, collapse_phase_a<W>(c, gi, raw->g[gi], R->g[gi], tmp[gi], dsample, S, dmeta, attempt, stage, dweight));
            if (k < 0) hc.lap("first kernel of the bulk group enqueued");
        }
        c->cur = c->stream;
        hc.lap("enqueue A");
        if (rc == -3 && attempt < 2) {
            (void)hipStreamSynchronize(c->aux); (void)hipStreamSynchronize(c->stream);
            for (int gi = 0; gi < MIRGE_NGROUPS; gi++) {
                collapse_tmp_release(c, tmp[gi]);
                ReadGroup& og = R->g[gi];
                c->release(og.seq); c->release(og.len); c->release(og.nmask); c->release(og.counts); c->release(og.first);
                og = ReadGroup();
            }
            c->flush_deferred();
            rc = 0; attempt = 1;
            continue;
        }
        bool hooked = false;
        if (rc == 0 && hook && hook->small_ready && attempt == 0 && tmp[big].partitioned && !c->overlap_mode) {
            uint32_t* const small = c->pinned + 512;
            hipError_t e = hipMemcpyAsync(small, dmeta, MIRGE_NGROUPS * 4, hipMemcpyDeviceToHost, c->aux);
            if (e == hipSuccess) e = hipEventRecord(c->ev_meta_small, c->aux);
            if (e == hipSuccess) e = hipEventRecord(c->ev_bulk_counted, c->stream);
            if (e == hipSuccess) {
                rc = hook->pre_sync(R.get(), tmp, dmeta, big);
                hooked = rc == 0;
            }
            if (e == hipSuccess && hooked) e = hipEventSynchronize(c->ev_meta_small);
            if (e == hipSuccess && hooked) {
                int xslot[MIRGE_NGROUPS];
                uint32_t n_small_u[MIRGE_NGROUPS];
                for (int gi = 0; gi < MIRGE_NGROUPS; gi++) n_small_u[gi] = gi == big ? 0u : small[gi];
                small_group_slots(n_small_u, big, big, xslot);
                bool forked = false;
                for (int gi = 0; gi < MIRGE_NGROUPS; gi++) forked |= xslot[gi] >= 0;
                for (int gi = 0; gi < MIRGE_NGROUPS; gi++)
                    if (gi != big && !is_long_group(gi) && small[gi] > small_fused_max()) forked = false;
                if (forked) rc = xaux_fork(c);
                for (int gi = 0; gi < MIRGE_NGROUPS && rc == 0; gi++) {
                    if (gi == big) continue;
                    c->cur = (forked && xslot[gi] >= 0) ? c->xaux[xslot[gi]] : c->aux;
                    if (is_long_group(gi)) rc = collapse_phase_b_long(c, gi, raw->g[gi], R->g[gi], tmp[gi], S, small[gi], 0u, dmeta);
                    else MIRGE_BY_WIDTH(gi, rc, collapse_phase_b<W>(c, gi, raw->g[gi], R->g[gi], tmp[gi], S, small[gi], 0u, dmeta));
                }
                c->cur = c->stream;
                c->xaux_forked = forked;
                if (rc == 0) { rc = hook->small_ready(R.get(), big); small_done = rc == 0; }
                c->xaux_forked = false;
            }
            if (e == hipSuccess) e = hipStreamWaitEvent(c->aux, c->ev_bulk_counted, 0);
            if (e == hipSuccess)
                for (int gi = 0; gi < MIRGE_NGROUPS; gi++) part_len_hist(c, R->g[gi], tmp[gi], dmeta, gi);
            if (e == hipSuccess) e = hipMemcpyAsync(c->pinned, dmeta, MIRGE_META_WORDS * 4, hipMemcpyDeviceToHost, c->aux);
            if (e == hipSuccess) e = hipEventRecord(c->ev_meta, c->aux);
            if (e == hipSuccess) e = hipEventSynchronize(c->ev_meta);
            if (e != hipSuccess && rc == 0) rc = fail(-2, std::string("mirge_collapse: ") + hipGetErrorString(e));
        } else
        if (rc == 0) {
            rc = stream_fork(c);
            if (rc == 0)
                for (int gi = 0; gi < MIRGE_NGROUPS; gi++) part_len_hist(c, R->g[gi], tmp[gi], dmeta, gi);
            hipError_t e = rc == 0 ? hipMemcpyAsync(c->pinned, dmeta, MIRGE_META_WORDS * 4, hipMemcpyDeviceToHost, c->aux) : hipErrorUnknown;
            if (e == hipSuccess) e = hipEventRecord(c->ev_meta, c->aux);
            if (e == hipSuccess && hook && attempt == 0 && tmp[big].partitioned) {
                rc = hook->pre_sync(R.get(), tmp, dmeta, big);
                hooked = rc == 0;
            }
            if (e == hipSuccess) e = hipEventSynchronize(c->ev_meta);
            if (e != hipSuccess && rc == 0) rc = fail(-2, std::string("mirge_collapse: ") + hipGetErrorString(e));
        }
        if (hooked && (rc != 0 || c->pinned[MIRGE_META_OVERFLOW])) { hook->discard(); hooked = false; small_done = false; }
        if (hook) { hook->ran = hooked; hook->small_ran = small_done; }
        if (rc == 0 && c->pinned[MIRGE_META_OVERFLOW] && attempt < 2) {
            for (int gi = 0; gi < MIRGE_NGROUPS; gi++) {
                collapse_tmp_release(c, tmp[gi]);
                ReadGroup& og = R->g[gi];
                c->release(og.seq); c->release(og.len); c->release(og.nmask); c->release(og.counts); c->release(og.first);
                og = ReadGroup();
            }
            c->flush_deferred();
            continue;
        }
        break;
    }
    hc.lap("sync");
    uint32_t base = 0;
    if (rc == 0) {
        uint32_t U[MIRGE_NGROUPS];
        for (int gi = 0; gi < MIRGE_NGROUPS; gi++) U[gi] = c->pinned[gi];
        R->total_bases = 0;
        for (int L = 0; L <= MIRGE_MAX_READ_LEN; L++) {
            R->len_hist[L] = (int32_t)c->pinned[MIRGE_META_HIST + L];
            R->total_bases += (int64_t)L * c->pinned[MIRGE_META_HIST + L];
        }
        R->total_bases += (int64_t)((uint64_t)c->pinned[MIRGE_META_LONG_BASES] | ((uint64_t)c->pinned[MIRGE_META_LONG_BASES + 1] << 32));
        R->long_max = raw->long_max;
        R->hist_valid = true;
        rc = stream_fork(c);
        for (int gi = 0; gi < MIRGE_NGROUPS && rc == 0; gi++) {
            c->cur = gi == big ? c->stream : c->aux;
            if (small_done && gi != big) R->g[gi].base = base;
            else if (is_long_group(gi)) rc = collapse_phase_b_long(c, gi, raw->g[gi], R->g[gi], tmp[gi], S, U[gi], base, dmeta);
            else MIRGE_BY_WIDTH(gi, rc, collapse_phase_b<W>(c, gi, raw->g[gi], R->g[gi], tmp[gi], S, U[gi], base, dmeta));
            base += R->g[gi].n;
        }
        c->cur = c->stream;
        if (!small_done) { int jr = stream_join(c); if (rc == 0) rc = jr; }
        else c->aux_drained = rc == 0;
    }
    for (int gi = 0; gi < MIRGE_NGROUPS; gi++) collapse_tmp_release(c, tmp[gi]);
    c->flush_deferred();
    c->release(dsample); c->release(dweight);
    if (rc && hook && hook->ran) { hook->discard(); hook->ran = false; }
    if (hook && hook->ran) hook->dmeta = dmeta;
    else c->release(dmeta);
    if (rc) { mirge_reads_destroy(R.release()); return rc; }
    R->n = base;
    *uniq = R.release();
    if (n_uniq) *n_uniq = base;
    hc.lap("phase B + release");
    return 0;
}

extern "C" int mirge_collapse_merge(mirge_ctx* c, const mirge_reads* const* parts, int32_t n_parts, mirge_reads** uniq, int64_t* n_uniq) {
    if (!c || !parts || n_parts < 1 || !uniq) return fail(-1, "mirge_collapse_merge: bad argument");
    HIPOK(hipSetDevice(c->device)); CHECK(join_pending_now(c));
    for (int p = 0; p < n_parts; p++) {
        if (!parts[p] || parts[p]->ctx != c || parts[p]->n_samples != 1) return fail(-1, "mirge_collapse_merge: every part must be a one-sample collapse result of this context");
        for (int gi = 0; gi < MIRGE_NGROUPS; gi++)
            if (parts[p]->g[gi].n && (parts[p]->g[gi].orig || !parts[p]->g[gi].counts)) return fail(-1, "mirge_collapse_merge: a part is not a collapse result");
    }
    mirge_reads* all = nullptr;
    CHECK(reads_concat_impl(c, parts, n_parts, &all, true));
    int32_t* dsample = nullptr;
    uint32_t* dweight = nullptr;
    int rc = dalloc(c, &dsample, (size_t)std::max<int64_t>(all->n, 1));
    if (rc == 0) rc = dalloc(c, &dweight, (size_t)std::max<int64_t>(all->n, 1));
    if (rc) { c->release(dsample); mirge_reads_destroy(all); return rc; }
    uint32_t before = 0;
    for (int p = 0; p < n_parts; p++) {
        for (int gi = 0; gi < MIRGE_NGROUPS; gi++) {
            const ReadGroup& g = parts[p]->g[gi];
            if (g.n) hipLaunchKernelGGL(k_merge_fill, dim3(grid_for(c, g.n)), dim3(MIRGE_BLOCK), 0, c->stream, (const uint32_t*)g.counts, g.n,
                                        before + g.base, (int32_t)p, dsample, dweight);
        }
        before += (uint32_t)parts[p]->n;
    }
    rc = collapse_impl(c, all, nullptr, n_parts, uniq, n_uniq, nullptr, nullptr, dsample, dweight);
    mirge_reads_destroy(all);
    return rc;
}

extern "C" int mirge_collapse_fetch(mirge_ctx* c, const mirge_reads* U, uint32_t* counts_out, int64_t* first_out) {
    if (!c || !U || !counts_out) return fail(-1, "mirge_collapse_fetch: bad argument");
    if (U->n_samples < 1) return fail(-1, "read set has no count matrix");
    HIPOK(hipSetDevice(c->device)); CHECK(join_pending_now(c));
    const int32_t S = U->n_samples;
    std::vector<uint32_t> tmp;
    for (int gi = 0; gi < MIRGE_NGROUPS; gi++) {
        const ReadGroup& g = U->g[gi];
        if (!g.n) continue;
        if (g.orig) return fail(-1, "mirge_collapse_fetch: handle is not a collapse result");
        HIPOK(hipMemcpyAsync(counts_out + (size_t)g.base * S, g.counts, (size_t)g.n * S * 4, hipMemcpyDeviceToHost, c->stream));
        if (first_out && g.first) {
            tmp.resize(g.n);
            HIPOK(hipMemcpyAsync(tmp.data(), g.first, (size_t)g.n * 4, hipMemcpyDeviceToHost, c->stream));
            HIPOK(hipStreamSynchronize(c->stream));
            for (uint32_t j = 0; j < g.n; j++) first_out[g.base + j] = tmp[j];
        }
    }
    HIPOK(hipStreamSynchronize(c->stream));
    return 0;
}

extern "C" int mirge_collapse_order(mirge_ctx* c, const mirge_reads* U, int64_t* order_out) {
    if (!c || !U || (!order_out && U->n)) return fail(-1, "mirge_collapse_order: bad argument");
    HIPOK(hipSetDevice(c->device)); CHECK(join_pending_now(c));
    const size_t n = (size_t)U->n;
    if (!n) return 0;
    if (n >= 0x7FFFFFFFull) return fail(-5, "mirge_collapse_order: 2^31 unique reads or more (hipCUB's sort takes an int count)");
    uint32_t *keys = nullptr, *vals = nullptr, *keys2 = nullptr, *vals2 = nullptr;
    CHECK(dalloc(c, &keys, n)); CHECK(dalloc(c, &vals, n)); CHECK(dalloc(c, &keys2, n)); CHECK(dalloc(c, &vals2, n));
    for (int gi = 0; gi < MIRGE_NGROUPS; gi++) {
        const ReadGroup& g = U->g[gi];
        if (!g.n) continue;
        if (g.orig || !g.first) return fail(-1, "mirge_collapse_order: handle is not a collapse result");
        HIPOK(hipMemcpyAsync(keys + g.base, g.first, (size_t)g.n * 4, hipMemcpyDeviceToDevice, c->stream));
        hipLaunchKernelGGL(k_index_shift, dim3(grid_for(c, g.n)), dim3(MIRGE_BLOCK), 0, c->stream, (const uint32_t*)nullptr, 0u,
                           (uint32_t)g.n, g.base, vals + g.base);
    }
    void* tmp = nullptr;
    size_t tmp_bytes = 0;
    HIPOK(hipcub::DeviceRadixSort::SortPairs(tmp, tmp_bytes, keys, keys2, vals, vals2, (int)n, 0, 32, c->stream));
    CHECK(dalloc(c, (uint8_t**)&tmp, std::max<size_t>(tmp_bytes, 16)));
    HIPOK(hipcub::DeviceRadixSort::SortPairs(tmp, tmp_bytes, keys, keys2, vals, vals2, (int)n, 0, 32, c->stream));
    std::vector<uint32_t> h(n);
    HIPOK(hipMemcpyAsync(h.data(), vals2, n * 4, hipMemcpyDeviceToHost, c->stream));
    HIPOK(hipStreamSynchronize(c->stream));
    for (size_t k = 0; k < n; k++) order_out[k] = (int64_t)h[k];
    c->release(keys); c->release(vals); c->release(keys2); c->release(vals2); c->release(tmp);
    return 0;
}
```

mirge3.0_amd/csrc/native_ctx.hpp:

```cpp
#pragma once
#define HIPOK(expr)                                                                          \
    do {                                                                                     \
        hipError_t _e = (expr);                                                              \
        if (_e != hipSuccess)                                                                \
            return fail(-2, std::string(#expr) + ": " + hipGetErrorString(_e));              \
    } while (0)

struct ProfRec {
    std::string name;
    int64_t launches = 0;
    double total_ms = 0.0;
    double units = 0.0;
};
struct PendingEvt {
    int rec;
    hipEvent_t a, b;
};
struct ProfUnits {
    int rec, stage;
    uint32_t grid;
    const uint32_t* host;
    double n_first;
};
#define MIRGE_PROF_PINNED_WORDS (1u << 18)

struct PassStep {
    int32_t p0 = 0, np = 1;
    const mirge_lib* lib = nullptr;
    MergeInfo mi;
    const MirgePlanTable* dplan = nullptr;
};

struct mirge_ctx {
    int device = 0;
    hipStream_t stream = nullptr;
    bool own_stream = false;
    hipStream_t aux = nullptr, cur = nullptr;
    hipEvent_t ev_fork = nullptr, ev_join = nullptr, ev_meta = nullptr, ev_meta_small = nullptr, ev_bulk_counted = nullptr;
#define MIRGE_N_SLOTS 2
#define MIRGE_N_XAUX 3
    hipStream_t xaux[MIRGE_N_XAUX] = {nullptr, nullptr, nullptr};
    hipEvent_t ev_xfork = nullptr, ev_xjoin[MIRGE_N_XAUX] = {nullptr, nullptr, nullptr};
    bool xaux_used = false;
    bool join_pending = false;
    bool overlap_mode = false;
    int n_cu = 256;
    std::multimap<size_t, void*> free_blocks;
    std::unordered_map<void*, size_t> sizes;
    size_t pool_bytes = 0;
    bool profiling = false;
    bool prof_units = true;
    std::string prof_only;
    std::vector<ProfRec> recs;
    std::unordered_map<std::string, int> rec_of;
    std::vector<PendingEvt> pending;
    std::vector<hipEvent_t> evt_pool;
    hipEvent_t t0 = nullptr, t1 = nullptr;
    uint32_t* pinned = nullptr;
    uint32_t* prof_pinned = nullptr;
    unsigned long long* join_pinned = nullptr;
    size_t join_pinned_bytes = 0;
    uint8_t* csv_pinned = nullptr;
    size_t csv_pinned_bytes = 0;
    uint8_t* sam_pinned = nullptr;
    size_t sam_pinned_bytes = 0;
    uint32_t* heavy_cnt = nullptr;
    bool x0_gathered = false, aux_drained = false;
    bool xaux_forked = false;
    uint32_t casc_big_t = 0;
    bool casc_rep = false;
    uint32_t* wg_pinned = nullptr;
    size_t wg_pinned_words = 0;
    uint32_t wg_grid = 0;
    unsigned long long* join_dev = nullptr;
    size_t join_dev_words = 0;
    bool join_dev_clean = false;
    struct PlanEntry { uint64_t uid; MirgePolicy pol; MirgePlanTable* dplan; };
    std::vector<PlanEntry> plans;
    struct FusedEntry { std::unique_ptr<FusedSteps> host; FusedSteps* dev; };
    std::vector<FusedEntry> fused;
    std::string casc_key;
    std::vector<PassStep> casc_steps;
    ResolveTable casc_rt;
    const FusedSteps* casc_dsteps = nullptr;
    struct WalksEntry { std::unique_ptr<BulkWalks> host; BulkWalks* dev; };
    std::vector<WalksEntry> walks;
    const BulkWalks* casc_dwalks[2] = {nullptr, nullptr};
    size_t prof_used = 0;
    std::vector<ProfUnits> prof_pending;

    int alloc(void** out, size_t bytes) {
        bytes = (std::max<size_t>(bytes, 1) + 255) & ~size_t(255);
        auto it = free_blocks.lower_bound(bytes);
        if (it != free_blocks.end() && it->first <= bytes * 2 + (1u << 20)) {
            *out = it->second;
            free_blocks.erase(it);
            return 0;
        }
        void* p = nullptr;
        hipError_t e = hipMalloc(&p, bytes);
        if (e != hipSuccess) {
            for (auto& kv : free_blocks) { (void)hipFree(kv.second); pool_bytes -= kv.first; sizes.erase(kv.second); }
            free_blocks.clear();
            e = hipMalloc(&p, bytes);
            if (e != hipSuccess) return fail(-3, "hipMalloc(" + std::to_string(bytes) + "): " + hipGetErrorString(e));
        }
        sizes[p] = bytes;
        pool_bytes += bytes;
        *out = p;
        return 0;
    }
    void release(void* p) {
        if (!p) return;
        auto it = sizes.find(p);
        if (it == sizes.end()) return;
        free_blocks.emplace(it->second, p);
    }
    struct Merged { std::vector<uint64_t> uids; struct mirge_lib* lib; };
    std::vector<Merged> merged;
    std::vector<void*> deferred;
    void defer(void* p) { if (p) deferred.push_back(p); }
    void flush_deferred() { if (overlap_mode) return; for (void* p : deferred) release(p); deferred.clear(); }
    int rec_index(const char* name) {
        auto it = rec_of.find(name);
        if (it != rec_of.end()) return it->second;
        recs.push_back(ProfRec{name});
        rec_of[name] = (int)recs.size() - 1;
        return (int)recs.size() - 1;
    }
    hipEvent_t get_evt() {
        if (!evt_pool.empty()) { hipEvent_t e = evt_pool.back(); evt_pool.pop_back(); return e; }
        hipEvent_t e; (void)hipEventCreate(&e); return e;
    }
    void drain() {
        for (auto& u : prof_pending) {
            double units = u.n_first;
            if (u.stage > 0) { units = 0; for (uint32_t b = 0; b < u.grid; b++) units += u.host[(size_t)u.grid * (u.stage - 1) + b]; }
            recs[u.rec].units += units;
        }
        prof_pending.clear();
        prof_used = 0;
        for (auto& p : pending) {
            float ms = 0.f;
            if (hipEventElapsedTime(&ms, p.a, p.b) == hipSuccess) recs[p.rec].total_ms += ms;
            evt_pool.push_back(p.a);
            evt_pool.push_back(p.b);
        }
        pending.clear();
    }
};

template <typename T>
static int dalloc(mirge_ctx* c, T** out, size_t count) { return c->alloc((void**)out, count * sizeof(T)); }

struct LaunchScope {
    mirge_ctx* c; int rec = -1; hipEvent_t a = nullptr, b = nullptr;
    LaunchScope(mirge_ctx* ctx, const char* name, double units) : c(ctx) {
        if (!c->profiling) return;
        if (!c->prof_only.empty() && !std::strstr(name, c->prof_only.c_str())) return;
        rec = c->rec_index(name);
        c->recs[rec].launches++;
        c->recs[rec].units += units;
        a = c->get_evt(); b = c->get_evt();
        (void)hipEventRecord(a, c->cur);
    }
    ~LaunchScope() {
        if (rec < 0) return;
        (void)hipEventRecord(b, c->cur);
        c->pending.push_back(PendingEvt{rec, a, b});
    }
};

static int stream_fork(mirge_ctx* c) {
    if (c->overlap_mode) return 0;
    HIPOK(hipEventRecord(c->ev_fork, c->stream));
    HIPOK(hipStreamWaitEvent(c->aux, c->ev_fork, 0));
    return 0;
}
static int xaux_fork(mirge_ctx* c) {
    HIPOK(hipEventRecord(c->ev_xfork, c->aux));
    for (int k = 0; k < MIRGE_N_XAUX; k++) HIPOK(hipStreamWaitEvent(c->xaux[k], c->ev_xfork, 0));
    c->xaux_used = true;
    return 0;
}
static int stream_join(mirge_ctx* c) {
    c->cur = c->stream;
    hipError_t e = hipSuccess;
    const bool x = c->xaux_used;
    const bool only_x0 = x && c->x0_gathered && c->aux_drained;
    c->x0_gathered = c->aux_drained = false;
    if (only_x0) {
        c->xaux_used = false;
        e = hipEventRecord(c->ev_xjoin[0], c->xaux[0]);
        if (e == hipSuccess) e = hipStreamWaitEvent(c->stream, c->ev_xjoin[0], 0);
        c->flush_deferred();
        if (e != hipSuccess) return fail(-2, std::string("stream join: ") + hipGetErrorString(e));
        return 0;
    }
    if (x) {
        for (int k = 1; k < MIRGE_N_XAUX && e == hipSuccess; k++) {
            e = hipEventRecord(c->ev_xjoin[k], c->xaux[k]);
            if (e == hipSuccess) e = hipStreamWaitEvent(c->aux, c->ev_xjoin[k], 0);
        }
        c->xaux_used = false;
    }
    if (e == hipSuccess) e = hipEventRecord(c->ev_join, c->aux);
    if (e == hipSuccess) e = hipStreamWaitEvent(c->stream, c->ev_join, 0);
    if (x && e == hipSuccess) {
        e = hipEventRecord(c->ev_xjoin[0], c->xaux[0]);
        if (e == hipSuccess) e = hipStreamWaitEvent(c->stream, c->ev_xjoin[0], 0);
    }
    c->flush_deferred();
    if (e != hipSuccess) return fail(-2, std::string("stream join: ") + hipGetErrorString(e));
    return 0;
}
static int join_pending_now(mirge_ctx* c) {
    if (!c->join_pending) return 0;
    c->join_pending = false;
    return stream_join(c);
}
static int largest_group(const struct mirge_reads* R);

static inline int grid_for(const mirge_ctx* c, size_t n, int per_block = MIRGE_BLOCK) {
    size_t blocks = (n + per_block - 1) / per_block;
    static const size_t per_cu = std::getenv("MIRGE_GRID_PER_CU") ? (size_t)std::atoi(std::getenv("MIRGE_GRID_PER_CU")) : 8;
    size_t cap = (size_t)c->n_cu * per_cu;
    return (int)std::max<size_t>(1, std::min(blocks, cap));
}

extern "C" int mirge_device_count(void) {
    int n = 0;
    if (hipGetDeviceCount(&n) != hipSuccess) return 0;
    return n;
}

extern "C" int mirge_ctx_create(int device, void* hip_stream, mirge_ctx** out) {
    if (!out) return fail(-1, "mirge_ctx_create: out is NULL");
    int n = mirge_device_count();
    if (n <= 0) return fail(-4, "no HIP device visible: the hot path has no CPU fallback");
    if (device < 0 || device >= n) return fail(-1, "device index out of range");
    HIPOK(hipSetDevice(device));
    auto c = std::make_unique<mirge_ctx>();
    c->device = device;
    hipDeviceProp_t prop;
    HIPOK(hipGetDeviceProperties(&prop, device));
    c->n_cu = prop.multiProcessorCount > 0 ? prop.multiProcessorCount : 256;
    if (hip_stream) { c->stream = (hipStream_t)hip_stream; }
    else { HIPOK(hipStreamCreateWithFlags(&c->stream, hipStreamNonBlocking)); c->own_stream = true; }
    c->cur = c->stream;
    HIPOK(hipStreamCreateWithFlags(&c->aux, hipStreamNonBlocking));
    for (int k = 0; k < MIRGE_N_XAUX; k++) {
        HIPOK(hipStreamCreateWithFlags(&c->xaux[k], hipStreamNonBlocking));
        HIPOK(hipEventCreateWithFlags(&c->ev_xjoin[k], hipEventDisableTiming));
    }
    HIPOK(hipEventCreateWithFlags(&c->ev_xfork, hipEventDisableTiming));
    HIPOK(hipEventCreateWithFlags(&c->ev_fork, hipEventDisableTiming));
    HIPOK(hipEventCreateWithFlags(&c->ev_join, hipEventDisableTiming));
    HIPOK(hipEventCreateWithFlags(&c->ev_meta, hipEventDisableTiming));
    HIPOK(hipEventCreateWithFlags(&c->ev_meta_small, hipEventDisableTiming));
    HIPOK(hipEventCreateWithFlags(&c->ev_bulk_counted, hipEventDisableTiming));
    HIPOK(hipEventCreate(&c->t0));
    HIPOK(hipEventCreate(&c->t1));
    HIPOK(hipHostMalloc((void**)&c->pinned, 4096, hipHostMallocDefault));
    HIPOK(hipHostMalloc((void**)&c->prof_pinned, MIRGE_PROF_PINNED_WORDS * 4, hipHostMallocDefault));
    *out = c.release();
    return 0;
}

extern "C" void mirge_lib_destroy(mirge_lib* L);
extern "C" void mirge_ctx_destroy(mirge_ctx* c) {
    if (!c) return;
    (void)hipSetDevice(c->device);
    (void)hipStreamSynchronize(c->stream);
    for (auto& m : c->merged) mirge_lib_destroy(m.lib);
    c->merged.clear();
    c->drain();
    for (auto& kv : c->sizes) (void)hipFree(kv.first);
    for (auto e : c->evt_pool) (void)hipEventDestroy(e);
    if (c->t0) (void)hipEventDestroy(c->t0);
    if (c->t1) (void)hipEventDestroy(c->t1);
    if (c->pinned) (void)hipHostFree(c->pinned);
    if (c->prof_pinned) (void)hipHostFree(c->prof_pinned);
    if (c->join_pinned) (void)hipHostFree(c->join_pinned);
    if (c->csv_pinned) (void)hipHostFree(c->csv_pinned);
    if (c->sam_pinned) (void)hipHostFree(c->sam_pinned);
    if (c->wg_pinned) (void)hipHostFree(c->wg_pinned);
    if (c->heavy_cnt) (void)hipFree(c->heavy_cnt);
    if (c->join_dev) (void)hipFree(c->join_dev);
    for (auto& e : c->plans) (void)hipFree(e.dplan);
    for (auto& e : c->fused) (void)hipFree(e.dev);
    for (auto& e : c->walks) (void)hipFree(e.dev);
    if (c->ev_fork) (void)hipEventDestroy(c->ev_fork);
    if (c->ev_join) (void)hipEventDestroy(c->ev_join);
    if (c->ev_meta) (void)hipEventDestroy(c->ev_meta);
    if (c->ev_meta_small) (void)hipEventDestroy(c->ev_meta_small);
    if (c->ev_bulk_counted) (void)hipEventDestroy(c->ev_bulk_counted);
    if (c->aux) (void)hipStreamDestroy(c->aux);
    for (int k = 0; k < MIRGE_N_XAUX; k++) {
        if (c->xaux[k]) (void)hipStreamDestroy(c->xaux[k]);
        if (c->ev_xjoin[k]) (void)hipEventDestroy(c->ev_xjoin[k]);
    }
    if (c->ev_xfork) (void)hipEventDestroy(c->ev_xfork);
    if (c->own_stream) (void)hipStreamDestroy(c->stream);
    delete c;
}

extern "C" int mirge_ctx_sync(mirge_ctx* c) {
    if (!c) return fail(-1, "ctx is NULL");
    HIPOK(hipSetDevice(c->device)); CHECK(join_pending_now(c));
    HIPOK(hipStreamSynchronize(c->stream));
    c->drain();
    return 0;
}

extern "C" int mirge_ctx_timer_start(mirge_ctx* c) {
    if (c) CHECK(join_pending_now(c));
    if (!c) return fail(-1, "ctx is NULL");
    HIPOK(hipEventRecord(c->t0, c->stream));
    return 0;
}
extern "C" int mirge_ctx_timer_stop(mirge_ctx* c, double* ms_out) {
    if (c) CHECK(join_pending_now(c));
    if (!c || !ms_out) return fail(-1, "NULL argument");
    HIPOK(hipEventRecord(c->t1, c->stream));
    HIPOK(hipEventSynchronize(c->t1));
    float ms = 0.f;
    HIPOK(hipEventElapsedTime(&ms, c->t0, c->t1));
    *ms_out = ms;
    return 0;
}
extern "C" int mirge_ctx_profile_enable(mirge_ctx* c, int32_t on) {
    if (!c) return fail(-1, "ctx is NULL");
    c->profiling = on != 0;
    return 0;
}
extern "C" int mirge_ctx_profile_only(mirge_ctx* c, const char* substr) {
    if (!c) return fail(-1, "ctx is NULL");
    c->prof_only = substr ? substr : "";
    return 0;
}
extern "C" int mirge_ctx_profile_units(mirge_ctx* c, int32_t on) {
    if (!c) return fail(-1, "ctx is NULL");
    c->prof_units = on != 0;
    return 0;
}
extern "C" int mirge_ctx_profile_reset(mirge_ctx* c) {
    if (!c) return fail(-1, "ctx is NULL");
    CHECK(mirge_ctx_sync(c));
    c->recs.clear();
    c->rec_of.clear();
    return 0;
}
extern "C" int32_t mirge_ctx_profile_count(mirge_ctx* c) {
    if (!c) return 0;
    if (mirge_ctx_sync(c) != 0) return 0;
    return (int32_t)c->recs.size();
}
extern "C" int mirge_ctx_profile_get(mirge_ctx* c, int32_t i, char* name_out, int32_t name_cap,
                                     int64_t* launches, double* total_ms, double* units) {
    if (!c || i < 0 || i >= (int32_t)c->recs.size()) return fail(-1, "profile index out of range");
    const ProfRec& r = c->recs[i];
    if (name_out && name_cap > 0) { std::snprintf(name_out, (size_t)name_cap, "%s", r.name.c_str()); }
    if (launches) *launches = r.launches;
    if (total_ms) *total_ms = r.total_ms;
    if (units) *units = r.units;
    return 0;
}
```

mirge3.0_amd/csrc/native_join.hpp:

```cpp
#pragma once
extern "C" int mirge_count_join(mirge_ctx* c, const mirge_reads* U, const mirge_result* res, int32_t exact_pass,
                                int32_t iso_pass, int64_t n_mirna, int64_t* class_sums, int64_t* exact, int64_t* iso) {
    HostClock hc("count_join");
    if (!c || !U || !res || !class_sums || !exact || !iso || n_mirna < 0) return fail(-1, "mirge_count_join: bad argument");
    if (U->n_samples < 1) return fail(-1, "read set has no count matrix (collapse it or mirge_reads_set_counts)");
    if (res->n != U->n) return fail(-1, "result and read set differ in size");
    for (int32_t p : {exact_pass, iso_pass})
        if (p >= 0 && p < res->n_pass && (int64_t)res->n_refs[p] > n_mirna)
            return fail(-1, "mirge_count_join: n_mirna (" + std::to_string(n_mirna) + ") is smaller than the " +
                                std::to_string(res->n_refs[p]) + " references of pass " + std::to_string(p));
    HIPOK(hipSetDevice(c->device));
    const int32_t S = U->n_samples, P = res->n_pass;
    const size_t n_cls = (size_t)P * S, n_tab = (size_t)std::max<int64_t>(n_mirna, 1) * S;
    const size_t words = n_cls + 2 * n_tab;
    if (c->join_dev_words < words) {
        if (c->join_dev) { HIPOK(hipStreamSynchronize(c->stream)); (void)hipFree(c->join_dev); }
        c->join_dev = nullptr; c->join_dev_words = 0; c->join_dev_clean = false;
        HIPOK(hipMalloc((void**)&c->join_dev, words * 8));
        c->join_dev_words = words;
    }
    unsigned long long* d = c->join_dev;
    if (!c->join_dev_clean) HIPOK(hipMemsetAsync(d, 0, c->join_dev_words * 8, c->stream));
    c->join_dev_clean = false;
    if (words * 8 > c->join_pinned_bytes) {
        if (c->join_pinned) { HIPOK(hipStreamSynchronize(c->stream)); (void)hipHostFree(c->join_pinned); }
        c->join_pinned = nullptr; c->join_pinned_bytes = 0;
        HIPOK(hipHostMalloc((void**)&c->join_pinned, words * 8 * 2, hipHostMallocDefault));
        c->join_pinned_bytes = words * 8 * 2;
    }
    unsigned long long* partial = nullptr;
    static const bool rows_off = std::getenv("MIRGE_JOIN_ROWS") && std::atoi(std::getenv("MIRGE_JOIN_ROWS")) == 0;
    const bool lazy = c->join_pending;
    auto join_side_streams = [&]() -> int {
        if (!lazy || !c->join_pending) return 0;
        c->join_pending = false;
        return stream_join(c);
    };
    struct PoolBlock {
        mirge_ctx* c; unsigned long long*& p;
        ~PoolBlock() { c->release(p); p = nullptr; }
    } partial_guard{c, partial};
    const int big = largest_group(U);
    auto group_list = [&](bool bulk, JoinGroups& gs) -> uint64_t {
        std::memset(&gs, 0, sizeof(gs));
        uint64_t total = 0;
        for (int gi = 0; gi < MIRGE_NGROUPS; gi++) {
            const ResGroup& g = res->g[gi];
            if (!g.n || (gi == big) != bulk) continue;
            gs.pass[gs.n_groups] = g.pass; gs.ref[gs.n_groups] = g.ref; gs.counts[gs.n_groups] = U->g[gi].counts;
            gs.start[gs.n_groups++] = (uint32_t)total;
            total += g.n;
        }
        gs.start[gs.n_groups] = (uint32_t)std::min<uint64_t>(total, 0xFFFFFFFFull);
        return total;
    };
    JoinGroups gb, gsm;
    const uint64_t n_bulk = group_list(true, gb), n_small = group_list(false, gsm);
    if (n_small >= 0xFFFFFFF0ull) return fail(-5, "mirge_count_join: more than 2^32 reads outside the bulk group");
    const bool by_rows = !rows_off && n_bulk + n_small >= 65536 && words <= MIRGE_JOIN_ROWS_CELLS && n_mirna * (int64_t)S < 0x7FFFFFFF;
    if (by_rows) {
        const uint32_t rows_b = n_bulk ? (uint32_t)std::min<uint64_t>((uint64_t)c->n_cu, (n_bulk + 4095) / 4096) : 0u;
        const uint32_t rows_s = n_small ? (uint32_t)std::min<uint64_t>((uint64_t)c->n_cu, (n_small + 4095) / 4096) : 0u;
        CHECK(dalloc(c, &partial, (size_t)(rows_b + rows_s) * words));
        if (rows_b) {
            LaunchScope ls(c, "k_join", (double)n_bulk);
            hipLaunchKernelGGL(k_join_rows, dim3(rows_b), dim3(MIRGE_JOIN_ROWS_THREADS), words * 8, c->stream, gb, S, P, exact_pass, iso_pass,
                               (uint32_t)n_tab, partial);
        }
        CHECK(join_side_streams());
        if (rows_s) {
            LaunchScope ls(c, "k_join", (double)n_small);
            hipLaunchKernelGGL(k_join_rows, dim3(rows_s), dim3(MIRGE_JOIN_ROWS_THREADS), words * 8, c->stream, gsm, S, P, exact_pass, iso_pass,
                               (uint32_t)n_tab, partial + (size_t)rows_b * words);
        }
        LaunchScope ls(c, "k_join_reduce", (double)words);
        hipLaunchKernelGGL(k_join_reduce, dim3((unsigned)((words + 63) / 64)), dim3(1024), 0, c->stream, partial, rows_b + rows_s, (uint32_t)words, d,
                           c->join_pinned);
    } else {
        CHECK(join_side_streams());
        for (JoinGroups* gs : {&gb, &gsm}) {
            const uint64_t total = gs == &gb ? n_bulk : n_small;
            if (!total) continue;
            LaunchScope ls(c, "k_join", (double)total);
            hipLaunchKernelGGL(k_join_multi, dim3(grid_for(c, (size_t)total)), dim3(MIRGE_BLOCK), 0, c->stream, *gs, S, P, exact_pass, iso_pass,
                               d, d + n_cls, d + n_cls + n_tab);
        }
    }
    bool cleared = true;
    if (!by_rows) {
        HIPOK(hipMemcpyAsync(c->join_pinned, d, words * 8, hipMemcpyDeviceToHost, c->stream));
    }
    HIPOK(hipEventRecord(c->ev_meta, c->stream));
    if (!by_rows) cleared = hipMemsetAsync(d, 0, c->join_dev_words * 8, c->stream) == hipSuccess;
    hc.lap("enqueue");
    HIPOK(hipEventSynchronize(c->ev_meta));
    hc.lap("wait for the tables");
    c->join_dev_clean = cleared;
    std::memcpy(class_sums, c->join_pinned, n_cls * 8);
    if (n_mirna) {
        std::memcpy(exact, c->join_pinned + n_cls, (size_t)n_mirna * S * 8);
        std::memcpy(iso, c->join_pinned + n_cls + n_tab, (size_t)n_mirna * S * 8);
    }
    c->drain();
    hc.lap("copy out + drain");
    return 0;
}

extern "C" int mirge_count_join_host(mirge_ctx* c, const int8_t* pass, const int32_t* ref, const uint32_t* counts,
                                     int64_t n, int32_t S, int32_t P, int32_t exact_pass, int32_t iso_pass,
                                     int64_t n_mirna, int64_t* class_sums, int64_t* exact, int64_t* iso) {
    if (!c || !class_sums || !exact || !iso || n < 0 || S < 1 || P < 1 || P > MIRGE_MAX_PASSES || n_mirna < 0 ||
        (n > 0 && (!pass || !ref || !counts)))
        return fail(-1, "mirge_count_join_host: bad argument");
    if (n >= 0xFFFFFFF0ll) return fail(-5, "more than 2^32 rows");
    HIPOK(hipSetDevice(c->device)); CHECK(join_pending_now(c));
    for (int64_t i = 0; i < n; i++) {
        if (pass[i] >= P) return fail(-1, "pass index out of range");
        if ((pass[i] == exact_pass || pass[i] == iso_pass) && (ref[i] < 0 || ref[i] >= n_mirna))
            return fail(-1, "miRNA reference index out of range");
    }
    const size_t n_cls = (size_t)P * S, n_tab = (size_t)std::max<int64_t>(n_mirna, 1) * S;
    unsigned long long* d = nullptr; int8_t* dp = nullptr; int32_t* dr = nullptr; uint32_t* dc = nullptr;
    CHECK(dalloc(c, &d, n_cls + 2 * n_tab));
    CHECK(dalloc(c, &dp, (size_t)std::max<int64_t>(n, 1)));
    CHECK(dalloc(c, &dr, (size_t)std::max<int64_t>(n, 1)));
    CHECK(dalloc(c, &dc, (size_t)std::max<int64_t>(n, 1) * S));
    HIPOK(hipMemsetAsync(d, 0, (n_cls + 2 * n_tab) * 8, c->stream));
    if (n) {
        HIPOK(hipMemcpyAsync(dp, pass, (size_t)n, hipMemcpyHostToDevice, c->stream));
        HIPOK(hipMemcpyAsync(dr, ref, (size_t)n * 4, hipMemcpyHostToDevice, c->stream));
        HIPOK(hipMemcpyAsync(dc, counts, (size_t)n * S * 4, hipMemcpyHostToDevice, c->stream));
        LaunchScope ls(c, "k_join", (double)n);
        hipLaunchKernelGGL(k_join, dim3(grid_for(c, (size_t)n)), dim3(MIRGE_BLOCK), 0, c->stream, dp, dr, dc, (uint32_t)n,
                           S, P, exact_pass, iso_pass, d, d + n_cls, d + n_cls + n_tab);
    }
    const size_t words = n_cls + 2 * n_tab;
    if (words * 8 > c->join_pinned_bytes) {
        if (c->join_pinned) (void)hipHostFree(c->join_pinned);
        c->join_pinned = nullptr; c->join_pinned_bytes = 0;
        HIPOK(hipHostMalloc((void**)&c->join_pinned, words * 8 * 2, hipHostMallocDefault));
        c->join_pinned_bytes = words * 8 * 2;
    }
    HIPOK(hipMemcpyAsync(c->join_pinned, d, words * 8, hipMemcpyDeviceToHost, c->stream));
    HIPOK(hipStreamSynchronize(c->stream));
    std::memcpy(class_sums, c->join_pinned, n_cls * 8);
    if (n_mirna) {
        std::memcpy(exact, c->join_pinned + n_cls, (size_t)n_mirna * S * 8);
        std::memcpy(iso, c->join_pinned + n_cls + n_tab, (size_t)n_mirna * S * 8);
    }
    c->drain();
    c->release(d); c->release(dp); c->release(dr); c->release(dc);
    return 0;
}

extern "C" int mirge_variant_tally(mirge_ctx* c, const mirge_reads* U, const mirge_result* res, int32_t exact_pass,
                                   int32_t iso_pass, const int32_t* fam_of_ref, int64_t n_mirna, const char* target_ascii,
                                   const int64_t* target_off, int64_t n_fam, const uint8_t* retained, const double* freq,
                                   int64_t* fam_tables, int64_t* census, int8_t* diag_out, int8_t* state_out) {
    static_assert(MIRGE_TALLY_POSITIONS == MIRGE_TALLY_MAXPOS, "tally positions");
    if (!c || !U || !res || !fam_of_ref || n_mirna < 0 || n_fam < 0 || !target_off || (n_fam > 0 && !target_ascii) || !freq ||
        !fam_tables || !census)
        return fail(-1, "mirge_variant_tally: bad argument");
    if (U->n_samples < 1) return fail(-1, "read set has no count matrix");
    if (res->n != U->n) return fail(-1, "result and read set differ in size");
    for (int32_t p : {exact_pass, iso_pass})
        if (p >= 0 && p < res->n_pass && (int64_t)res->n_refs[p] > n_mirna)
            return fail(-1, "mirge_variant_tally: fam_of_ref is shorter than the miRNA library of pass " + std::to_string(p));
    HIPOK(hipSetDevice(c->device)); CHECK(join_pending_now(c));
    const int32_t S = U->n_samples;
    std::vector<uint64_t> tb((size_t)std::max<int64_t>(n_fam, 1), 0ull);
    std::vector<uint8_t> tl((size_t)std::max<int64_t>(n_fam, 1), 0);
    for (int64_t f = 0; f < n_fam; f++) {
        const int64_t L = target_off[f + 1] - target_off[f];
        if (L < 0 || L > MIRGE_TALLY_MAXPOS) return fail(-6, "family " + std::to_string(f) + ": canonical sequence of " + std::to_string(L) + " nt; the limit is 32");
        for (int64_t k = 0; k < L; k++) {
            const int code = mirge_base_code(target_ascii[target_off[f] + k]);
            if (code < 0) return fail(-7, "family " + std::to_string(f) + ": canonical sequence holds a character other than A/C/G/T/U");
            tb[(size_t)f] |= (uint64_t)code << (2 * k);
        }
        tl[(size_t)f] = (uint8_t)L;
    }
    for (int64_t r = 0; r < n_mirna; r++)
        if (fam_of_ref[r] >= n_fam) return fail(-1, "fam_of_ref holds a family index out of range");
    const size_t n_fs = (size_t)std::max<int64_t>(n_fam, 1) * S, n_cen = n_fs * MIRGE_TALLY_MAXPOS * 16 * 3;
    const size_t n_words = 5 * n_fs + n_cen;
    unsigned long long* d = nullptr;
    uint64_t* dtb = nullptr; uint8_t* dtl = nullptr; int32_t* dfam = nullptr; uint8_t* dret = nullptr; double* dfreq = nullptr;
    int8_t *ddiag = nullptr, *dstate = nullptr;
    const size_t n = (size_t)std::max<int64_t>(U->n, 1);
    CHECK(dalloc(c, &d, n_words));
    CHECK(dalloc(c, &dtb, tb.size()));
    CHECK(dalloc(c, &dtl, tl.size()));
    CHECK(dalloc(c, &dfam, (size_t)std::max<int64_t>(n_mirna, 1)));
    CHECK(dalloc(c, &dfreq, (size_t)S));
    CHECK(dalloc(c, &ddiag, n));
    CHECK(dalloc(c, &dstate, n));
    if (retained) CHECK(dalloc(c, &dret, n));
    HIPOK(hipMemsetAsync(d, 0, n_words * 8, c->stream));
    HIPOK(hipMemcpyAsync(dtb, tb.data(), tb.size() * 8, hipMemcpyHostToDevice, c->stream));
    HIPOK(hipMemcpyAsync(dtl, tl.data(), tl.size(), hipMemcpyHostToDevice, c->stream));
    if (n_mirna) HIPOK(hipMemcpyAsync(dfam, fam_of_ref, (size_t)n_mirna * 4, hipMemcpyHostToDevice, c->stream));
    HIPOK(hipMemcpyAsync(dfreq, freq, (size_t)S * 8, hipMemcpyHostToDevice, c->stream));
    if (retained && U->n) HIPOK(hipMemcpyAsync(dret, retained, (size_t)U->n, hipMemcpyHostToDevice, c->stream));
    HIPOK(hipMemsetAsync(dstate, 0xFF, n, c->stream));
    HIPOK(hipMemsetAsync(ddiag, 0, n, c->stream));
    TallyOut o;
    o.n_seqs = d; o.seq_true = d + n_fs; o.count_true = d + 2 * n_fs; o.canon = d + 3 * n_fs; o.kept_exact = d + 4 * n_fs;
    o.census = d + 5 * n_fs; o.diag = ddiag; o.state = dstate;
    std::vector<uint32_t*> lists;
    for (int gi = 0; gi < MIRGE_NGROUPS; gi++) {
        if (kGroupW[gi] != 1) continue;
        const ResGroup& g = res->g[gi];
        const ReadGroup& rg = U->g[gi];
        if (!g.n) continue;
        const uint32_t tgrid = (uint32_t)grid_for(c, g.n);
        uint32_t chunk = ((uint32_t)g.n + tgrid - 1) / tgrid;
        chunk = (chunk + MIRGE_BLOCK - 1) / MIRGE_BLOCK * MIRGE_BLOCK;
        uint32_t* dlist = nullptr;
        CHECK(dalloc(c, &dlist, (size_t)tgrid * chunk + tgrid));
        uint32_t* dnlist = dlist + (size_t)tgrid * chunk;
        {
            LaunchScope ls(c, "k_member_list", g.n);
            const TallyMember pred{g.pass, g.ref, rg.counts, S, exact_pass, iso_pass, dfam, dfreq};
            hipLaunchKernelGGL((k_member_list<TallyMember, MIRGE_BLOCK>), dim3(tgrid), dim3(MIRGE_BLOCK), 0, c->stream, (uint32_t)g.n, chunk,
                               pred, dlist, dnlist);
        }
        LaunchScope ls(c, "k_tally", g.n);
        hipLaunchKernelGGL(k_tally, dim3(tgrid), dim3(MIRGE_BLOCK), 0, c->stream, view_of<1>(rg), rg.base,
                           (const uint32_t*)rg.orig, g.pass, g.ref, rg.counts, S, exact_pass, iso_pass, dfam, dtb, dtl,
                           (const uint8_t*)dret, dfreq, o, (const uint32_t*)dlist, (const uint32_t*)dnlist, chunk);
        lists.push_back(dlist);
    }
    for (int t = 0; t < 5 && n_fam; t++)
        HIPOK(hipMemcpyAsync(fam_tables + (size_t)t * n_fam * S, d + (size_t)t * n_fs, (size_t)n_fam * S * 8, hipMemcpyDeviceToHost, c->stream));
    if (n_fam) HIPOK(hipMemcpyAsync(census, d + 5 * n_fs, (size_t)n_fam * S * MIRGE_TALLY_MAXPOS * 16 * 3 * 8, hipMemcpyDeviceToHost, c->stream));
    if (diag_out && U->n) HIPOK(hipMemcpyAsync(diag_out, ddiag, (size_t)U->n, hipMemcpyDeviceToHost, c->stream));
    if (state_out && U->n) HIPOK(hipMemcpyAsync(state_out, dstate, (size_t)U->n, hipMemcpyDeviceToHost, c->stream));
    HIPOK(hipStreamSynchronize(c->stream));
    c->drain();
    c->release(d); c->release(dtb); c->release(dtl); c->release(dfam); c->release(dret); c->release(dfreq);
    c->release(ddiag); c->release(dstate);
    for (uint32_t* l : lists) c->release(l);
    return 0;
}
```

mirge3.0_amd/csrc/native_lib.hpp:

```cpp
#pragma once
static std::atomic<uint64_t> g_lib_uid{1};

struct mirge_lib {
    mirge_ctx* ctx = nullptr;
    uint64_t uid = 0;
    MirgeHostLib h;
    uint64_t* dT = nullptr;
    uint64_t* dinv = nullptr;
    uint32_t* dref_start = nullptr;
    uint32_t* dcoarse = nullptr;
    MirgeKTable* dtables = nullptr;
    std::vector<MirgeKTable> htables;
    size_t device_bytes = 0;
    std::mutex mu;
    int64_t n_refs = 0;
    int kmax = 8;
    uint32_t max_bucket = 0;
    struct ExactTab { uint64_t* slots = nullptr; uint32_t mask = 0; uint64_t windows = 0; };
    std::map<uint32_t, ExactTab> exact;

    MirgeLibView view() const {
        MirgeLibView v;
        v.T = dT; v.inv = dinv; v.ref_start = dref_start; v.tables = dtables;
        v.total = h.total; v.n_refs = (uint32_t)n_refs; v.kmax = kmax;
        return v;
    }
};

static int lib_upload(mirge_ctx* c, std::unique_ptr<mirge_lib>& L, int64_t n_refs, mirge_lib** out);

extern "C" int mirge_lib_create(mirge_ctx* c, const char* seq, const int64_t* off, int64_t n_refs, mirge_lib** out) {
    if (!c || !out || (!seq && n_refs > 0) || !off || n_refs < 0) return fail(-1, "mirge_lib_create: bad argument");
    HIPOK(hipSetDevice(c->device)); CHECK(join_pending_now(c));
    auto L = std::make_unique<mirge_lib>();
    L->ctx = c;
    L->uid = g_lib_uid.fetch_add(1);
    std::string err;
    int rc = mirge_hostlib_build(L->h, seq, off, n_refs, err);
    if (rc) return fail(rc, "mirge_lib_create: " + err);
    return lib_upload(c, L, n_refs, out);
}

extern "C" int mirge_lib_create_packed(mirge_ctx* c, const uint64_t* T, int64_t n_T, const uint64_t* inv, int64_t n_inv,
                                       const uint32_t* ref_start, int64_t n_refs, uint64_t total, int32_t kmax,
                                       uint64_t valid_positions, mirge_lib** out) {
    if (!c || !out) return fail(-1, "mirge_lib_create_packed: bad argument");
    CHECK(lib_packed_args_check(T, n_T, inv, n_inv, ref_start, n_refs, total, kmax));
    HIPOK(hipSetDevice(c->device)); CHECK(join_pending_now(c));
    auto L = std::make_unique<mirge_lib>();
    L->ctx = c;
    L->uid = g_lib_uid.fetch_add(1);
    L->h.n_refs = n_refs; L->h.total = total; L->h.kmax = kmax; L->h.valid_positions = valid_positions;
    L->h.T.assign(T, T + n_T);
    L->h.inv.assign(inv, inv + n_inv);
    L->h.ref_start.assign(ref_start, ref_start + n_refs + 1);
    return lib_upload(c, L, n_refs, out);
}
extern "C" int mirge_lib_packed_sizes(const mirge_lib* L, int64_t* sizes, int32_t* kmax) {
    if (!L || !sizes || !kmax) return fail(-1, "mirge_lib_packed_sizes: bad argument");
    sizes[0] = (int64_t)L->h.T.size(); sizes[1] = (int64_t)L->h.inv.size(); sizes[2] = (int64_t)L->h.total; sizes[3] = (int64_t)L->h.valid_positions;
    *kmax = L->h.kmax;
    return 0;
}
extern "C" int mirge_lib_packed_copy(const mirge_lib* L, uint64_t* T, uint64_t* inv, uint32_t* ref_start) {
    if (!L || !T || !inv || !ref_start) return fail(-1, "mirge_lib_packed_copy: bad argument");
    std::memcpy(T, L->h.T.data(), L->h.T.size() * 8);
    std::memcpy(inv, L->h.inv.data(), L->h.inv.size() * 8);
    std::memcpy(ref_start, L->h.ref_start.data(), L->h.ref_start.size() * 4);
    return 0;
}

static int lib_upload(mirge_ctx* c, std::unique_ptr<mirge_lib>& L, int64_t n_refs, mirge_lib** out) {
    L->n_refs = n_refs;
    L->kmax = L->h.kmax;
    L->htables.assign(MIRGE_SHAPE_SLOTS, MirgeKTable{nullptr, nullptr, nullptr});
    const size_t nT = L->h.T.size() * 8, nI = L->h.inv.size() * 8, nR = ((size_t)n_refs + 1) * 4;
    HIPOK(hipMalloc((void**)&L->dT, nT));
    HIPOK(hipMalloc((void**)&L->dinv, nI));
    HIPOK(hipMalloc((void**)&L->dref_start, nR));
    HIPOK(hipMalloc((void**)&L->dtables, sizeof(MirgeKTable) * MIRGE_SHAPE_SLOTS));
    HIPOK(hipMemcpy(L->dT, L->h.T.data(), nT, hipMemcpyHostToDevice));
    HIPOK(hipMemcpy(L->dinv, L->h.inv.data(), nI, hipMemcpyHostToDevice));
    HIPOK(hipMemcpy(L->dref_start, L->h.ref_start.data(), nR, hipMemcpyHostToDevice));
    HIPOK(hipMemcpy(L->dtables, L->htables.data(), sizeof(MirgeKTable) * MIRGE_SHAPE_SLOTS, hipMemcpyHostToDevice));
    size_t nC = 0;
    if (n_refs > 0) {
        const size_t n_gran = (size_t)(L->h.total >> MIRGE_COARSE_SHIFT) + 2;
        if ((uint64_t)n_refs >= (1ull << 27)) return fail(-1, "mirge_lib_create: more than 2^27 references");
        std::vector<uint32_t> coarse(2 * n_gran);
        const std::vector<uint32_t>& rs = L->h.ref_start;
        uint32_t t = 0;
        for (size_t b = 0; b < n_gran; b++) {
            const uint64_t x = (uint64_t)b << MIRGE_COARSE_SHIFT, xe = x + (1ull << MIRGE_COARSE_SHIFT);
            while ((int64_t)t + 1 < n_refs && rs[(size_t)t + 1] <= x) t++;
            uint32_t inside = 0;
            while ((int64_t)t + 1 + inside < n_refs && rs[(size_t)t + 1 + inside] < xe) inside++;
            const uint32_t code = inside == 0 ? 16u : inside == 1 ? (uint32_t)(rs[(size_t)t + 1] - x) : 17u;
            coarse[2 * b] = t << 5 | code;
            coarse[2 * b + 1] = rs[t];
        }
        nC = coarse.size() * 4;
        HIPOK(hipMalloc((void**)&L->dcoarse, nC));
        HIPOK(hipMemcpy(L->dcoarse, coarse.data(), nC, hipMemcpyHostToDevice));
    }
    L->device_bytes = nT + nI + nR + nC + sizeof(MirgeKTable) * MIRGE_SHAPE_SLOTS;
    *out = L.release();
    return 0;
}

extern "C" void mirge_lib_destroy(mirge_lib* L) {
    if (!L) return;
    (void)hipSetDevice(L->ctx->device);
    (void)hipStreamSynchronize(L->ctx->stream);
    (void)hipFree(L->dT); (void)hipFree(L->dinv); (void)hipFree(L->dref_start); (void)hipFree(L->dcoarse); (void)hipFree(L->dtables);
    for (auto& t : L->htables) { (void)hipFree((void*)t.bucket); (void)hipFree((void*)t.pos); (void)hipFree((void*)((uintptr_t)t.bits & ~(uintptr_t)3)); }
    for (auto& e : L->exact) (void)hipFree(e.second.slots);
    delete L;
}
extern "C" int64_t mirge_lib_n_refs(const mirge_lib* L) { return L ? L->n_refs : -1; }
extern "C" int64_t mirge_lib_device_bytes(const mirge_lib* L) { return L ? (int64_t)L->device_bytes : -1; }

struct ShapeJob {
    int k1 = 0, gap = 0, k2 = 0;
};

static int lib_build_shapes(mirge_lib* L, const std::vector<ShapeJob>& jobs) {
    mirge_ctx* c = L->ctx;
    struct Built { int sid; uint64_t nb; uint32_t *A, *dpos, *dbits; uint64_t* dentry; };
    std::vector<Built> built;
    void* tmp = nullptr;
    uint32_t* A_scratch = nullptr;
    size_t tmp_cap = 0;
    uint64_t nb_max = 0, nb_scratch = 0;
    for (const ShapeJob& j : jobs) {
        const uint64_t nb = 1ull << (2 * (j.k1 + j.k2));
        nb_max = std::max(nb_max, nb);
        if (j.k1 + j.k2 > MIRGE_BITMAP_MAXK) nb_scratch = std::max(nb_scratch, nb);
    }
    hipError_t e = hipcub::DeviceScan::InclusiveSum(nullptr, tmp_cap, (uint32_t*)nullptr, (uint32_t*)nullptr, (int)(nb_max + 2), c->stream);
    if (e == hipSuccess) e = hipMalloc(&tmp, std::max<size_t>(tmp_cap, 16));
    if (e == hipSuccess && nb_scratch) e = hipMalloc((void**)&A_scratch, (nb_scratch + 2) * 4);
    const int grid = c->n_cu * 8;
    const uint32_t heavy_cap = (uint32_t)std::min<uint64_t>(L->h.total / (MIRGE_LIGHT_MAX + 1) + 16, 0x7FFFFFF0ull);
    uint32_t *seg_begin = nullptr, *seg_end = nullptr, *n_heavy = nullptr, *pos_sorted = nullptr;
    void* sort_tmp = nullptr;
    size_t sort_tmp_cap = 0;
    const bool sort_heavy = true;
    int pos_bits = 1;
    while (pos_bits < 32 && (1ull << pos_bits) < L->h.total + 1) pos_bits++;
    if (e == hipSuccess && sort_heavy && !jobs.empty()) {
        e = hipMalloc((void**)&seg_begin, (size_t)heavy_cap * 4);
        if (e == hipSuccess) e = hipMalloc((void**)&seg_end, (size_t)heavy_cap * 4);
        if (e == hipSuccess) e = hipMalloc((void**)&n_heavy, 64);
        if (e == hipSuccess) e = hipMalloc((void**)&pos_sorted, std::max<size_t>((size_t)L->h.total, 1) * 4);
    }
    for (size_t k = 0; k < jobs.size() && e == hipSuccess; k++) {
        const ShapeJob& j = jobs[k];
        Built t{mirge_shape_id(j.k1, j.gap, j.k2), 1ull << (2 * (j.k1 + j.k2)), nullptr, nullptr, nullptr, nullptr};
        const uint64_t nb = t.nb;
        const bool entries = j.k1 + j.k2 > MIRGE_BITMAP_MAXK;
        if (!entries) e = hipMalloc((void**)&t.A, (nb + 2) * 4);
        if (e == hipSuccess) e = hipMalloc((void**)&t.dpos, std::max<size_t>((size_t)L->h.total, 1) * 4);
        if (e == hipSuccess && (!entries || MIRGE_PRESENCE_FILTER)) e = hipMalloc((void**)&t.dbits, (size_t)((nb + 31) / 32) * 4);
        if (e == hipSuccess && entries) e = hipMalloc((void**)&t.dentry, nb * 8);
        built.push_back(t);
        uint32_t* A = entries ? A_scratch : t.A;
        if (e == hipSuccess) e = hipMemsetAsync(A, 0, (nb + 2) * 4, c->stream);
        if (e != hipSuccess) break;
        hipLaunchKernelGGL(k_table_pass<false>, dim3(grid), dim3(MIRGE_BLOCK), 0, c->stream, L->dT, L->dinv, L->h.total, j.k1,
                           j.gap, j.k2, A, (uint32_t*)nullptr);
        size_t tb = tmp_cap;
        e = hipcub::DeviceScan::InclusiveSum(tmp, tb, A, A, (int)(nb + 2), c->stream);
        if (e != hipSuccess) break;
        hipLaunchKernelGGL(k_table_pass<true>, dim3(grid), dim3(MIRGE_BLOCK), 0, c->stream, L->dT, L->dinv, L->h.total, j.k1,
                           j.gap, j.k2, A, t.dpos);
        if (sort_heavy && L->h.total > MIRGE_LIGHT_MAX) {
            uint32_t nh = 0;
            e = hipMemsetAsync(n_heavy, 0, 8, c->stream);
            if (e != hipSuccess) break;
            hipLaunchKernelGGL(k_table_heavy_list, dim3(grid_for(c, (size_t)std::min<uint64_t>(nb, 1ull << 24))), dim3(MIRGE_BLOCK), 0, c->stream,
                               (const uint32_t*)A, nb, (uint32_t)MIRGE_LIGHT_MAX + 1u, n_heavy, heavy_cap, seg_begin, seg_end,
                               (uint32_t)std::min<uint64_t>(0xFFFFFFFFull, std::max<uint64_t>(1024, 32 * (L->h.total / nb + 1))));
            uint32_t nh2[2] = {0, 0};
            e = hipMemcpyAsync(nh2, n_heavy, 8, hipMemcpyDeviceToHost, c->stream);
            if (e == hipSuccess) e = hipStreamSynchronize(c->stream);
            if (e != hipSuccess) break;
            nh = std::min(nh2[0], heavy_cap);
            L->max_bucket = std::max(L->max_bucket, nh2[1]);
            if (nh) {
                size_t need = 0;
                e = hipcub::DeviceSegmentedRadixSort::SortKeys(nullptr, need, (const uint32_t*)t.dpos, pos_sorted, (int)std::min<uint64_t>(L->h.total, 0x7FFFFFFFull),
                                                               (int)nh, seg_begin, seg_end, 0, pos_bits, c->stream);
                if (e == hipSuccess && need > sort_tmp_cap) {
                    (void)hipFree(sort_tmp); sort_tmp = nullptr; sort_tmp_cap = 0;
                    e = hipMalloc(&sort_tmp, need + need / 4 + 256);
                    if (e == hipSuccess) sort_tmp_cap = need + need / 4 + 256;
                }
                size_t tb2 = sort_tmp_cap;
                if (e == hipSuccess)
                    e = hipcub::DeviceSegmentedRadixSort::SortKeys(sort_tmp, tb2, (const uint32_t*)t.dpos, pos_sorted, (int)std::min<uint64_t>(L->h.total, 0x7FFFFFFFull),
                                                                   (int)nh, seg_begin, seg_end, 0, pos_bits, c->stream);
                if (e != hipSuccess) break;
                hipLaunchKernelGGL(k_table_heavy_copy, dim3((unsigned)std::min<uint32_t>(nh, (uint32_t)c->n_cu * 16u)), dim3(MIRGE_BLOCK), 0, c->stream,
                                   (const uint32_t*)seg_begin, (const uint32_t*)seg_end, nh, (const uint32_t*)pos_sorted, t.dpos);
            }
        }
        if (!entries || MIRGE_PRESENCE_FILTER)
            hipLaunchKernelGGL(k_table_bits, dim3(grid_for(c, (size_t)((nb + 31) / 32))), dim3(MIRGE_BLOCK), 0, c->stream, A, nb, t.dbits);
        if (entries)
            hipLaunchKernelGGL(k_table_entries, dim3(grid_for(c, nb)), dim3(MIRGE_BLOCK), 0, c->stream, A, t.dpos, nb, t.dentry);
    }
    { const hipError_t e2 = hipStreamSynchronize(c->stream); if (e == hipSuccess) e = e2; }
    if (e == hipSuccess) e = hipGetLastError();
    (void)hipFree(tmp);
    (void)hipFree(A_scratch);
    (void)hipFree(seg_begin); (void)hipFree(seg_end); (void)hipFree(n_heavy); (void)hipFree(pos_sorted); (void)hipFree(sort_tmp);
    if (e != hipSuccess) {
        for (auto& t : built) { (void)hipFree(t.A); (void)hipFree(t.dpos); (void)hipFree(t.dbits); (void)hipFree(t.dentry); }
        return fail(e == hipErrorOutOfMemory ? -3 : -2, std::string("probe table construction: ") + hipGetErrorString(e));
    }
    for (const Built& t : built) {
        L->device_bytes += (t.dentry ? t.nb * 8 : (t.nb + 2) * 4) + (size_t)L->h.total * 4 + (t.dbits ? (size_t)((t.nb + 31) / 32) * 4 : 0);
        L->htables[t.sid].bucket = t.dentry ? (const void*)t.dentry : (const void*)t.A;
        L->htables[t.sid].pos = t.dpos;
        L->htables[t.sid].bits = (t.dentry && t.dbits) ? (const uint32_t*)((uintptr_t)t.dbits | 1u) : t.dbits;
    }
    if (!built.empty())
        HIPOK(hipMemcpy(L->dtables, L->htables.data(), sizeof(MirgeKTable) * MIRGE_SHAPE_SLOTS, hipMemcpyHostToDevice));
    return 0;
}

static int lib_prepare_shapes(mirge_lib* L, const std::vector<ShapeJob>& wanted) {
    std::lock_guard<std::mutex> lk(L->mu);
    std::vector<ShapeJob> jobs;
    std::vector<int> seen;
    for (const auto& w : wanted) {
        if (w.k1 < 1 || w.k2 < 0 || w.k1 + w.k2 > (w.k2 == 0 ? MIRGE_KMAX0 : MIRGE_KMAX) || w.gap < 0 || w.gap > 31 || (w.k2 == 0 && w.gap != 0))
            return fail(-1, "probe shape out of range");
        const int sid = mirge_shape_id(w.k1, w.gap, w.k2);
        if (L->htables[sid].bucket || std::find(seen.begin(), seen.end(), sid) != seen.end()) continue;
        seen.push_back(sid);
        jobs.push_back(w);
    }
    if (jobs.empty()) return 0;
    HIPOK(hipSetDevice(L->ctx->device));
    return lib_build_shapes(L, jobs);
}

#ifndef MIRGE_EXACT_MAX_WINDOWS
#define MIRGE_EXACT_MAX_WINDOWS (4u << 20)
#endif
static bool lib_exact_trim(mirge_lib* L) {
    std::lock_guard<std::mutex> lk(L->mu);
    if (L->exact.size() < 6) return false;
    (void)hipSetDevice(L->ctx->device);
    (void)hipDeviceSynchronize();
    for (auto& e : L->exact)
        if (e.second.slots) { L->device_bytes -= ((size_t)e.second.mask + 1) * 8; (void)hipFree(e.second.slots); }
    L->exact.clear();
    return true;
}

static int lib_exact_table(mirge_lib* L, uint32_t lmask, mirge_lib::ExactTab* out) {
    *out = mirge_lib::ExactTab();
    lmask &= 0xFFFFFFFEu;
    if (!lmask) return 0;
    std::lock_guard<std::mutex> lk(L->mu);
    auto it = L->exact.find(lmask);
    if (it != L->exact.end()) { *out = it->second; return 0; }
    mirge_ctx* c = L->ctx;
    HIPOK(hipSetDevice(c->device));
    mirge_lib::ExactTab tab;
    if ((uint64_t)__builtin_popcount(lmask) * L->h.valid_positions <= 4ull * MIRGE_EXACT_MAX_WINDOWS) {
        unsigned long long* dcount = nullptr;
        HIPOK(hipMalloc((void**)&dcount, 8));
        HIPOK(hipMemsetAsync(dcount, 0, 8, c->stream));
        const int grid = (int)std::min<uint64_t>((uint64_t)c->n_cu * 8, std::max<uint64_t>(1, (L->h.total + MIRGE_BLOCK - 1) / MIRGE_BLOCK));
        hipLaunchKernelGGL(k_exact_table<false>, dim3(grid), dim3(MIRGE_BLOCK), 0, c->stream, L->dT, L->dinv, L->h.total, lmask,
                           (uint64_t*)nullptr, 0u, dcount);
        unsigned long long n = 0;
        hipError_t e = hipMemcpyAsync(&n, dcount, 8, hipMemcpyDeviceToHost, c->stream);
        if (e == hipSuccess) e = hipStreamSynchronize(c->stream);
        (void)hipFree(dcount);
        if (e != hipSuccess) return fail(-2, std::string("exact table (count): ") + hipGetErrorString(e));
        tab.windows = n;
        if (n <= MIRGE_EXACT_MAX_WINDOWS) {
            uint64_t ns = 1024;
            while (ns < 3 * n) ns <<= 1;
            e = hipMalloc((void**)&tab.slots, ns * 8);
            if (e == hipSuccess) e = hipMemsetAsync(tab.slots, 0, ns * 8, c->stream);
            if (e == hipSuccess) {
                tab.mask = (uint32_t)(ns - 1);
                hipLaunchKernelGGL(k_exact_table<true>, dim3(grid), dim3(MIRGE_BLOCK), 0, c->stream, L->dT, L->dinv, L->h.total, lmask,
                                   tab.slots, tab.mask, (unsigned long long*)nullptr);
                e = hipStreamSynchronize(c->stream);
                if (e == hipSuccess) e = hipGetLastError();
            }
            if (e != hipSuccess) {
                (void)hipFree(tab.slots);
                return fail(e == hipErrorOutOfMemory ? -3 : -2, std::string("exact table: ") + hipGetErrorString(e));
            }
            L->device_bytes += ns * 8;
        }
    }
    L->exact[lmask] = tab;
    *out = tab;
    return 0;
}

extern "C" int mirge_lib_prepare(mirge_lib* L, int32_t k) {
    if (!L) return fail(-1, "lib is NULL");
    std::vector<ShapeJob> w(1);
    w[0].k1 = k;
    return lib_prepare_shapes(L, w);
}
```

Before: 8344.

## Defer big-group resolve and fuse ref lookup into join kernels

For the largest group, the k_resolve launch is deferred. The join kernels then compute miRNA reference ids directly from positions via the coarse/ref_start tables, and only for exact/iso passes. The deferred resolve runs after the join's event record, or earlier when the library epoch changed, so it leaves the critical path before the host wait. The change also reorders small-group scheduling and stream slots so speculative small groups avoid slots holding fused groups. It adds bookkeeping for a library epoch and pending state, which brings lifetime and ordering risks.

```diff
diff --git a/mirge3.0_amd/csrc/kernels_join.hpp b/mirge3.0_amd/csrc/kernels_join.hpp
--- a/mirge3.0_amd/csrc/kernels_join.hpp
+++ b/mirge3.0_amd/csrc/kernels_join.hpp
@@ -31,13 +31,31 @@
     }
 }
 
+struct JoinResolveRow { const uint32_t* ref_start; const uint32_t* coarse; uint32_t n_refs; };
 struct JoinGroups {
     const int8_t* pass[MIRGE_NCLS];
     const int32_t* ref[MIRGE_NCLS];
+    const uint32_t* pos[MIRGE_NCLS];
     const uint32_t* counts[MIRGE_NCLS];
     uint32_t start[MIRGE_NCLS + 1];
     int32_t n_groups;
+    int32_t from_pos;
+    JoinResolveRow mi[2];
 };
+__device__ __forceinline__ PairU32 join_granule(const JoinResolveRow& t, uint32_t g) {
+    return load_pair32((gptr_u32)t.coarse + 2 * (size_t)(g >> MIRGE_COARSE_SHIFT));
+}
+__device__ __forceinline__ uint32_t join_ref_at(const JoinResolveRow& t, const PairU32 e, uint32_t g) {
+    int32_t ref, off;
+    resolve_entry(e, t.ref_start, t.n_refs, g, ref, off);
+    return (uint32_t)ref;
+}
+__device__ __forceinline__ uint32_t join_ref(const JoinGroups& gs, bool is_iso, const int32_t* gr, const uint32_t* gq, uint32_t i) {
+    if (!gs.from_pos) return (uint32_t)gr[i];
+    const JoinResolveRow t = is_iso ? gs.mi[1] : gs.mi[0];
+    const uint32_t g = gq[i];
+    return join_ref_at(t, join_granule(t, g), g);
+}
 __global__ void k_join_multi(JoinGroups gs, int32_t S, int32_t n_pass, int32_t exact_pass, int32_t iso_pass,
                              unsigned long long* __restrict__ class_sums, unsigned long long* __restrict__ exact,
                              unsigned long long* __restrict__ iso) {
@@ -54,12 +72,13 @@
 #pragma unroll
         for (int q = 1; q < MIRGE_NCLS; q++) if (q < gs.n_groups && t >= gs.start[q]) k = q;
         const uint32_t i = t - gs.start[k];
-        const int8_t* gp = nullptr; const int32_t* gr = nullptr; const uint32_t* gc = nullptr;
-#pragma unroll
-        for (int q = 0; q < MIRGE_NCLS; q++) if (q == k) { gp = gs.pass[q]; gr = gs.ref[q]; gc = gs.counts[q]; }
+        const int8_t* gp = nullptr; const int32_t* gr = nullptr; const uint32_t* gq = nullptr; const uint32_t* gc = nullptr;
+#pragma unroll
+        for (int q = 0; q < MIRGE_NCLS; q++) if (q == k) { gp = gs.pass[q]; gr = gs.ref[q]; gq = gs.pos[q]; gc = gs.counts[q]; }
         const int p = gp[i];
         if (p < 0) continue;
-        const int32_t ref = gr[i];
+        const bool mirna = p == exact_pass || p == iso_pass;
+        const uint32_t ref = mirna ? join_ref(gs, p != exact_pass, gr, gq, i) : 0u;
         for (int32_t s = 0; s < S; s++) {
             const unsigned long long c = gc[(size_t)i * S + s];
             if (!c) continue;
@@ -88,6 +107,8 @@
     const uint32_t total = gs.start[gs.n_groups];
     if (gs.n_groups == 1 && S == 1) {
         const int8_t* __restrict__ gp = gs.pass[0]; const int32_t* __restrict__ gr = gs.ref[0]; const uint32_t* __restrict__ gc = gs.counts[0];
+        const uint32_t* __restrict__ gq = gs.pos[0];
+        const bool from_pos = gs.from_pos != 0;
         const uint64_t stride = (uint64_t)gridDim.x * blockDim.x;
         for (uint64_t t0 = (uint64_t)blockIdx.x * blockDim.x + threadIdx.x; t0 < total; t0 += 4 * stride) {
             int p[4]; uint32_t r[4]; unsigned long long c[4];
@@ -96,8 +117,19 @@
                 const uint64_t i = t0 + (uint64_t)u * stride;
                 const bool in = i < total;
                 p[u] = in ? (int)gp[i] : -1;
-                r[u] = in ? (uint32_t)gr[i] : 0u;
+                r[u] = in ? (from_pos ? gq[i] : (uint32_t)gr[i]) : 0u;
                 c[u] = in ? (unsigned long long)gc[i] : 0ull;
+            }
+            if (from_pos) {
+                PairU32 e[4]; bool m[4];
+#pragma unroll
+                for (int u = 0; u < 4; u++) {
+                    m[u] = p[u] >= 0 && (p[u] == exact_pass || p[u] == iso_pass);
+                    e[u] = m[u] ? join_granule(p[u] == exact_pass ? gs.mi[0] : gs.mi[1], r[u]) : PairU32{0u, 0u};
+                }
+#pragma unroll
+                for (int u = 0; u < 4; u++)
+                    if (m[u]) r[u] = join_ref_at(p[u] == exact_pass ? gs.mi[0] : gs.mi[1], e[u], r[u]);
             }
 #pragma unroll
             for (int u = 0; u < 4; u++) {
@@ -112,13 +144,14 @@
         int k = 0;
 #pragma unroll
         for (int q = 1; q < MIRGE_NCLS; q++) if (q < gs.n_groups && t >= gs.start[q]) k = q;
-        const int8_t* gp = gs.pass[0]; const int32_t* gr = gs.ref[0]; const uint32_t* gc = gs.counts[0];
-#pragma unroll
-        for (int q = 1; q < MIRGE_NCLS; q++) if (q == k) { gp = gs.pass[q]; gr = gs.ref[q]; gc = gs.counts[q]; }
+        const int8_t* gp = gs.pass[0]; const int32_t* gr = gs.ref[0]; const uint32_t* gq = gs.pos[0]; const uint32_t* gc = gs.counts[0];
+#pragma unroll
+        for (int q = 1; q < MIRGE_NCLS; q++) if (q == k) { gp = gs.pass[q]; gr = gs.ref[q]; gq = gs.pos[q]; gc = gs.counts[q]; }
         const uint32_t i = t - gs.start[k];
         const int p = gp[i];
         if (p < 0) continue;
-        const uint32_t ref = (uint32_t)gr[i];
+        const bool mirna = p == exact_pass || p == iso_pass;
+        const uint32_t ref = mirna ? join_ref(gs, p != exact_pass, gr, gq, i) : 0u;
         for (int32_t s = 0; s < S; s++) {
             const unsigned long long c = gc[(size_t)i * S + s];
             if (!c) continue;
diff --git a/mirge3.0_amd/csrc/native_cascade.hpp b/mirge3.0_amd/csrc/native_cascade.hpp
--- a/mirge3.0_amd/csrc/native_cascade.hpp
+++ b/mirge3.0_amd/csrc/native_cascade.hpp
@@ -15,6 +15,8 @@
     const mirge_reads* reads = nullptr;
     uint32_t n_refs[MIRGE_MAX_PASSES] = {0};
     uint32_t* dmeta = nullptr;
+    ResolveTable rt;
+    uint64_t lib_epoch = ~0ull;
 };
 
 extern "C" void mirge_result_destroy(mirge_result* r) {
@@ -101,7 +103,8 @@
 template <int W>
 static int cascade_group(mirge_ctx* c, const ReadGroup& rg, ResGroup& out, const std::vector<PassStep>& steps,
                          const mirge_policy* pol, const ResolveTable& rt, const char* gtag,
-                         const uint32_t* n_dev = nullptr, uint32_t n_cap = 0, const BulkWalks* dwalks = nullptr) {
+                         const uint32_t* n_dev = nullptr, uint32_t n_cap = 0, const BulkWalks* dwalks = nullptr, bool defer_resolve = false) {
+    defer_resolve = defer_resolve && c->casc_libs_own;
     out.n = n_dev ? 0 : rg.n;
     if (!n_dev && !rg.n) return 0;
     const uint32_t n = n_dev ? n_cap : rg.n;
@@ -142,6 +145,7 @@
     uint32_t* act_out = actA;
     int stage = 0;
     char name[32];
+    const uint32_t* wg_src = nullptr;
     std::vector<std::pair<int, int>> stage_of_pass;
     static const bool bulk_fused = !(std::getenv("MIRGE_BULK_FUSED") && std::atoi(std::getenv("MIRGE_BULK_FUSED")) == 0);
     if (bulk_fused && dwalks && steps.size() > 1) {
@@ -158,12 +162,13 @@
         stage = (int)steps.size();
         if (c->profiling && W == 1) {
             if (c->wg_pinned_words < 2 * (size_t)grid) {
-                if (c->wg_pinned) (void)hipHostFree(c->wg_pinned);
+                if (c->wg_pinned) { HIPOK(hipStreamSynchronize(c->stream)); (void)hipHostFree(c->wg_pinned); }
                 c->wg_pinned = nullptr; c->wg_pinned_words = 0;
                 if (hipHostMalloc((void**)&c->wg_pinned, 2 * (size_t)grid * 4, hipHostMallocDefault) == hipSuccess) c->wg_pinned_words = 2 * (size_t)grid;
             }
-            if (c->wg_pinned_words >= 2 * (size_t)grid) {
-                HIPOK(hipMemcpyAsync(c->wg_pinned, seg_n + (size_t)grid * (MIRGE_MAX_PASSES + 1), 2 * (size_t)grid * 4, hipMemcpyDeviceToHost, c->cur));
+            if (c->wg_pinned_words >= 2 * (size_t)grid) wg_src = seg_n + (size_t)grid * (MIRGE_MAX_PASSES + 1);
+            if (wg_src && !defer_resolve) {
+                HIPOK(hipMemcpyAsync(c->wg_pinned, wg_src, 2 * (size_t)grid * 4, hipMemcpyDeviceToHost, c->cur));
                 c->wg_grid = grid;
             }
         }
@@ -203,8 +208,15 @@
         stage++;
     }
     if (hcnt && stage > 0) launch_heavy<W>(c, rg, out, c->casc_dsteps, rt, gtag, hcnt, hlist, v, false);
-    {
-        std::snprintf(name, sizeof(name), "k_resolve%s", gtag);
+    std::snprintf(name, sizeof(name), "k_resolve%s", gtag);
+    if (defer_resolve) {
+        CHECK(resolve_pending_now(c));
+        mirge_ctx::PendingResolve& r = c->resolve_pending;
+        r.rt = rt; r.pass = out.pass; r.pos = out.pos; r.n = n; r.ref = out.ref; r.off = out.off; r.n_dev = n_dev;
+        std::snprintf(r.name, sizeof(r.name), "%s", name);
+        r.wg_src = wg_src; r.wg_grid = grid;
+        r.set = true;
+    } else {
         LaunchScope ls(c, name, n);
         hipLaunchKernelGGL(k_resolve, dim3(grid_for(c, n)), dim3(MIRGE_BLOCK), 0, c->cur, rt, out.pass, out.pos, n, out.ref, out.off, n_dev);
     }
@@ -236,9 +248,8 @@
     uint32_t* hlist = nullptr;
     if (hcnt) CHECK(dalloc(c, &hlist, (size_t)n));
     char name[32];
-    static const uint32_t spec_max = std::getenv("MIRGE_SPEC_MAX") ? (uint32_t)std::strtoul(std::getenv("MIRGE_SPEC_MAX"), nullptr, 10) : 32768u;
     const int nsteps = (int)c->casc_steps.size();
-    if (n <= spec_max && nsteps > 1) {
+    if (n <= small_spec_max(c)) {
         unsigned long long* answers = nullptr;
         const uint32_t rounds = (n + MIRGE_BLOCK - 1) / MIRGE_BLOCK, stride = rounds * MIRGE_BLOCK;
         CHECK(dalloc(c, &answers, (size_t)nsteps * stride));
@@ -297,6 +308,8 @@
                            const BulkWalks** dwalks_out) {
     for (int p = 0; p < MIRGE_MAX_PASSES; p++) { rt.ref_start[p] = nullptr; rt.coarse[p] = nullptr; rt.n_refs[p] = 0; }
     steps.clear();
+    c->casc_libs_own = true;
+    for (int32_t p = 0; p < n_pass; p++) if (libs[p] && libs[p]->ctx != c) c->casc_libs_own = false;
     for (int32_t p = 0; p < n_pass; p++) {
         if (!libs[p]) continue;
         if (libs[p]->ctx->device != c->device) return fail(-1, "library lives on another device");
@@ -500,14 +513,23 @@
     int rc = 0;
     const int big = big_is >= 0 ? big_is : largest_group(R);
     CHECK(stream_fork(c));
-    int order[MIRGE_NGROUPS], no = 0;
-    for (int gi = 0; gi < MIRGE_NGROUPS; gi++) if (gi != big) order[no++] = gi;
-    std::stable_sort(order, order + no, [&](int a, int b) { return R->g[a].n > R->g[b].n; });
-    order[no++] = big;
     uint32_t n[MIRGE_NGROUPS];
     int slot[MIRGE_NGROUPS];
     for (int gi = 0; gi < MIRGE_NGROUPS; gi++) n[gi] = R->g[gi].n;
-    if (small_group_slots(n, big, skip, slot) && !c->xaux_forked) CHECK(xaux_fork(c));
+    const uint32_t spec_max = small_spec_max(c);
+    if (small_group_slots(n, big, skip, slot, spec_max) && !c->xaux_forked) CHECK(xaux_fork(c));
+    auto rank = [&](int gi) {
+        if (is_long_group(gi) || n[gi] > fused_max) return 1;
+        return n[gi] <= spec_max ? 2 : 3;
+    };
+    int order[MIRGE_NGROUPS], no = 0;
+    for (int gi = 0; gi < MIRGE_NGROUPS; gi++) if (gi != big) order[no++] = gi;
+    std::stable_sort(order, order + no, [&](int a, int b) {
+        const int ra = rank(a), rb = rank(b);
+        if (ra != rb) return ra < rb;
+        return ra == 3 ? n[a] < n[b] : n[a] > n[b];
+    });
+    order[no++] = big;
     for (int k = 0; k < MIRGE_NGROUPS && rc == 0; k++) {
         const int gi = order[k];
         if (gi == skip) continue;
@@ -521,7 +543,7 @@
             MIRGE_BY_WIDTH(gi, rc, cascade_group_fused<W>(c, R->g[gi], res->g[gi], dsteps, rt, group_tag(gi)));
             continue;
         }
-        MIRGE_BY_WIDTH(gi, rc, cascade_group<W>(c, R->g[gi], res->g[gi], steps, pol, rt, group_tag(gi), nullptr, 0, c->casc_dwalks[W == 1 ? 0 : 1]));
+        MIRGE_BY_WIDTH(gi, rc, cascade_group<W>(c, R->g[gi], res->g[gi], steps, pol, rt, group_tag(gi), nullptr, 0, c->casc_dwalks[W == 1 ? 0 : 1], gi == big));
     }
     c->x0_gathered = false;
     if (rc == 0 && c->xaux_forked && c->xaux_used) {
@@ -562,6 +584,7 @@
     hc.lap("plans+fused");
     auto res = std::make_unique<mirge_result>();
     res->ctx = c; res->n = R->n; res->n_pass = n_pass; res->reads = R;
+    res->rt = c->casc_rt; res->lib_epoch = g_lib_epoch.load();
     for (int32_t p = 0; p < n_pass; p++) res->n_refs[p] = libs[p] ? (uint32_t)libs[p]->n_refs : 0u;
     const int rc = cascade_launch_groups(c, R, res.get(), pol, -1);
     hc.lap("enqueue+join");
@@ -623,6 +646,7 @@
     CHECK(cascade_config(c, libs, pol, n_pass, raw->len_hist, raw->long_max > 0));
     auto res = std::make_unique<mirge_result>();
     res->ctx = c; res->n_pass = n_pass;
+    res->rt = c->casc_rt; res->lib_epoch = g_lib_epoch.load();
     for (int32_t p = 0; p < n_pass; p++) res->n_refs[p] = libs[p] ? (uint32_t)libs[p]->n_refs : 0u;
     const size_t prof_mark = c->prof_pending.size();
     int hooked_group = -1;
@@ -631,7 +655,7 @@
         ReadGroup rg = partial->g[big];
         rg.n = raw->g[big].n;
         c->cur = c->stream;
-        const int rc = cascade_group<1>(c, rg, res->g[big], c->casc_steps, pol, c->casc_rt, group_tag(big), dmeta + big, raw->g[big].n, c->casc_dwalks[0]);
+        const int rc = cascade_group<1>(c, rg, res->g[big], c->casc_steps, pol, c->casc_rt, group_tag(big), dmeta + big, raw->g[big].n, c->casc_dwalks[0], true);
         if (rc == 0) { hooked_group = big; c->overlap_mode = true; }
         return rc;
     };
@@ -643,6 +667,7 @@
         (void)hipStreamSynchronize(c->aux);
         for (int k = 0; k < MIRGE_N_XAUX; k++) (void)hipStreamSynchronize(c->xaux[k]);
         c->overlap_mode = false;
+        c->resolve_pending.set = false;
         c->join_pending = false;
         c->xaux_used = false;
         c->x0_gathered = c->aux_drained = false;
diff --git a/mirge3.0_amd/csrc/native_collapse.hpp b/mirge3.0_amd/csrc/native_collapse.hpp
--- a/mirge3.0_amd/csrc/native_collapse.hpp
+++ b/mirge3.0_amd/csrc/native_collapse.hpp
@@ -324,7 +324,11 @@
     static const uint32_t v = std::getenv("MIRGE_FUSED_MAX") ? (uint32_t)std::strtoul(std::getenv("MIRGE_FUSED_MAX"), nullptr, 10) : (1u << 19);
     return v;
 }
-static bool small_group_slots(const uint32_t* n, int big, int skip, int* slot) {
+static uint32_t small_spec_max(const mirge_ctx* c) {
+    static const uint32_t v = std::getenv("MIRGE_SPEC_MAX") ? (uint32_t)std::strtoul(std::getenv("MIRGE_SPEC_MAX"), nullptr, 10) : 32768u;
+    return c->casc_steps.size() > 1 ? v : 0u;
+}
+static bool small_group_slots(const uint32_t* n, int big, int skip, int* slot, uint32_t spec_max) {
     const uint32_t fused_max = small_fused_max();
     int order[MIRGE_NGROUPS], no = 0;
     for (int gi = 0; gi < MIRGE_NGROUPS; gi++) { slot[gi] = -1; if (gi != big && gi != skip) order[no++] = gi; }
@@ -333,10 +337,21 @@
     for (int k = 0; k < no; k++) if (n[order[k]] && n[order[k]] <= fused_max) n_small++;
     if (n_small <= 1) return false;
     int next = 0;
+    bool holds_fused[MIRGE_N_SLOTS] = {false};
     for (int k = 0; k < no; k++) {
         const int gi = order[k];
-        if (is_long_group(gi) || !n[gi] || n[gi] > fused_max) continue;
+        if (is_long_group(gi) || !n[gi] || n[gi] > fused_max || n[gi] <= spec_max) continue;
         slot[gi] = next++ % MIRGE_N_SLOTS;
+        holds_fused[slot[gi]] = true;
+    }
+    int n_free = 0;
+    for (int q = 0; q < MIRGE_N_SLOTS; q++) n_free += holds_fused[q] ? 0 : 1;
+    for (int k = 0; k < no; k++) {
+        const int gi = order[k];
+        if (is_long_group(gi) || !n[gi] || n[gi] > fused_max || n[gi] > spec_max) continue;
+        int q = next++ % MIRGE_N_SLOTS;
+        while (n_free && holds_fused[q]) q = next++ % MIRGE_N_SLOTS;
+        slot[gi] = q;
     }
     return true;
 }
@@ -417,7 +432,7 @@
                 int xslot[MIRGE_NGROUPS];
                 uint32_t n_small_u[MIRGE_NGROUPS];
                 for (int gi = 0; gi < MIRGE_NGROUPS; gi++) n_small_u[gi] = gi == big ? 0u : small[gi];
-                small_group_slots(n_small_u, big, big, xslot);
+                small_group_slots(n_small_u, big, big, xslot, small_spec_max(c));
                 bool forked = false;
                 for (int gi = 0; gi < MIRGE_NGROUPS; gi++) forked |= xslot[gi] >= 0;
                 for (int gi = 0; gi < MIRGE_NGROUPS; gi++)
diff --git a/mirge3.0_amd/csrc/native_ctx.hpp b/mirge3.0_amd/csrc/native_ctx.hpp
--- a/mirge3.0_amd/csrc/native_ctx.hpp
+++ b/mirge3.0_amd/csrc/native_ctx.hpp
@@ -82,12 +82,21 @@
     std::string casc_key;
     std::vector<PassStep> casc_steps;
     ResolveTable casc_rt;
+    bool casc_libs_own = false;
     const FusedSteps* casc_dsteps = nullptr;
     struct WalksEntry { std::unique_ptr<BulkWalks> host; BulkWalks* dev; };
     std::vector<WalksEntry> walks;
     const BulkWalks* casc_dwalks[2] = {nullptr, nullptr};
     size_t prof_used = 0;
     std::vector<ProfUnits> prof_pending;
+    struct PendingResolve {
+        bool set = false;
+        ResolveTable rt;
+        const int8_t* pass = nullptr; const uint32_t* pos = nullptr; uint32_t n = 0;
+        int32_t* ref = nullptr; int32_t* off = nullptr; const uint32_t* n_dev = nullptr;
+        char name[32] = {0};
+        const uint32_t* wg_src = nullptr; uint32_t wg_grid = 0;
+    } resolve_pending;
 
     int alloc(void** out, size_t bytes) {
         bytes = (std::max<size_t>(bytes, 1) + 255) & ~size_t(255);
@@ -140,13 +149,17 @@
         }
         prof_pending.clear();
         prof_used = 0;
+        std::vector<PendingEvt> later;
         for (auto& p : pending) {
             float ms = 0.f;
-            if (hipEventElapsedTime(&ms, p.a, p.b) == hipSuccess) recs[p.rec].total_ms += ms;
+            const hipError_t e = hipEventElapsedTime(&ms, p.a, p.b);
+            if (e == hipErrorNotReady) { later.push_back(p); continue; }
+            if (e == hipSuccess) recs[p.rec].total_ms += ms;
             evt_pool.push_back(p.a);
             evt_pool.push_back(p.b);
         }
-        pending.clear();
+        if (!later.empty()) (void)hipGetLastError();
+        pending.swap(later);
     }
 };
 
@@ -214,14 +227,33 @@
     if (e != hipSuccess) return fail(-2, std::string("stream join: ") + hipGetErrorString(e));
     return 0;
 }
+static inline int grid_for(const mirge_ctx* c, size_t n, int per_block = MIRGE_BLOCK);
+static int resolve_pending_now(mirge_ctx* c) {
+    mirge_ctx::PendingResolve& r = c->resolve_pending;
+    if (!r.set) return 0;
+    r.set = false;
+    hipStream_t const cur = c->cur;
+    c->cur = c->stream;
+    {
+        LaunchScope ls(c, r.name, r.n);
+        hipLaunchKernelGGL(k_resolve, dim3(grid_for(c, r.n)), dim3(MIRGE_BLOCK), 0, c->stream, r.rt, r.pass, r.pos, r.n, r.ref, r.off, r.n_dev);
+    }
+    c->cur = cur;
+    if (r.wg_src) {
+        HIPOK(hipMemcpyAsync(c->wg_pinned, r.wg_src, 2 * (size_t)r.wg_grid * 4, hipMemcpyDeviceToHost, c->stream));
+        c->wg_grid = r.wg_grid;
+    }
+    return 0;
+}
 static int join_pending_now(mirge_ctx* c) {
+    CHECK(resolve_pending_now(c));
     if (!c->join_pending) return 0;
     c->join_pending = false;
     return stream_join(c);
 }
 static int largest_group(const struct mirge_reads* R);
 
-static inline int grid_for(const mirge_ctx* c, size_t n, int per_block = MIRGE_BLOCK) {
+static inline int grid_for(const mirge_ctx* c, size_t n, int per_block) {
     size_t blocks = (n + per_block - 1) / per_block;
     static const size_t per_cu = std::getenv("MIRGE_GRID_PER_CU") ? (size_t)std::atoi(std::getenv("MIRGE_GRID_PER_CU")) : 8;
     size_t cap = (size_t)c->n_cu * per_cu;
diff --git a/mirge3.0_amd/csrc/native_join.hpp b/mirge3.0_amd/csrc/native_join.hpp
--- a/mirge3.0_amd/csrc/native_join.hpp
+++ b/mirge3.0_amd/csrc/native_join.hpp
@@ -41,13 +41,21 @@
         ~PoolBlock() { c->release(p); p = nullptr; }
     } partial_guard{c, partial};
     const int big = largest_group(U);
+    const bool from_pos = res->ctx == c && res->lib_epoch == g_lib_epoch.load();
     auto group_list = [&](bool bulk, JoinGroups& gs) -> uint64_t {
         std::memset(&gs, 0, sizeof(gs));
+        gs.from_pos = from_pos ? 1 : 0;
+        const int32_t mirna_pass[2] = {exact_pass, iso_pass};
+        for (int k = 0; k < 2 && from_pos; k++) {
+            const int32_t p = mirna_pass[k];
+            if (p < 0 || p >= res->n_pass) continue;
+            gs.mi[k].ref_start = res->rt.ref_start[p]; gs.mi[k].coarse = res->rt.coarse[p]; gs.mi[k].n_refs = res->rt.n_refs[p];
+        }
         uint64_t total = 0;
         for (int gi = 0; gi < MIRGE_NGROUPS; gi++) {
             const ResGroup& g = res->g[gi];
             if (!g.n || (gi == big) != bulk) continue;
-            gs.pass[gs.n_groups] = g.pass; gs.ref[gs.n_groups] = g.ref; gs.counts[gs.n_groups] = U->g[gi].counts;
+            gs.pass[gs.n_groups] = g.pass; gs.ref[gs.n_groups] = g.ref; gs.pos[gs.n_groups] = g.pos; gs.counts[gs.n_groups] = U->g[gi].counts;
             gs.start[gs.n_groups++] = (uint32_t)total;
             total += g.n;
         }
@@ -62,6 +70,7 @@
         const uint32_t rows_b = n_bulk ? (uint32_t)std::min<uint64_t>((uint64_t)c->n_cu, (n_bulk + 4095) / 4096) : 0u;
         const uint32_t rows_s = n_small ? (uint32_t)std::min<uint64_t>((uint64_t)c->n_cu, (n_small + 4095) / 4096) : 0u;
         CHECK(dalloc(c, &partial, (size_t)(rows_b + rows_s) * words));
+        if (!from_pos) CHECK(resolve_pending_now(c));
         if (rows_b) {
             LaunchScope ls(c, "k_join", (double)n_bulk);
             hipLaunchKernelGGL(k_join_rows, dim3(rows_b), dim3(MIRGE_JOIN_ROWS_THREADS), words * 8, c->stream, gb, S, P, exact_pass, iso_pass,
@@ -77,6 +86,7 @@
         hipLaunchKernelGGL(k_join_reduce, dim3((unsigned)((words + 63) / 64)), dim3(1024), 0, c->stream, partial, rows_b + rows_s, (uint32_t)words, d,
                            c->join_pinned);
     } else {
+        if (!from_pos) CHECK(resolve_pending_now(c));
         CHECK(join_side_streams());
         for (JoinGroups* gs : {&gb, &gsm}) {
             const uint64_t total = gs == &gb ? n_bulk : n_small;
@@ -91,6 +101,7 @@
         HIPOK(hipMemcpyAsync(c->join_pinned, d, words * 8, hipMemcpyDeviceToHost, c->stream));
     }
     HIPOK(hipEventRecord(c->ev_meta, c->stream));
+    CHECK(resolve_pending_now(c));
     if (!by_rows) cleared = hipMemsetAsync(d, 0, c->join_dev_words * 8, c->stream) == hipSuccess;
     hc.lap("enqueue");
     HIPOK(hipEventSynchronize(c->ev_meta));
diff --git a/mirge3.0_amd/csrc/native_lib.hpp b/mirge3.0_amd/csrc/native_lib.hpp
--- a/mirge3.0_amd/csrc/native_lib.hpp
+++ b/mirge3.0_amd/csrc/native_lib.hpp
@@ -1,5 +1,6 @@
 #pragma once
 static std::atomic<uint64_t> g_lib_uid{1};
+static std::atomic<uint64_t> g_lib_epoch{0};
 
 struct mirge_lib {
     mirge_ctx* ctx = nullptr;
@@ -111,6 +112,8 @@
 extern "C" void mirge_lib_destroy(mirge_lib* L) {
     if (!L) return;
     (void)hipSetDevice(L->ctx->device);
+    (void)resolve_pending_now(L->ctx);
+    g_lib_epoch.fetch_add(1);
     (void)hipStreamSynchronize(L->ctx->stream);
     (void)hipFree(L->dT); (void)hipFree(L->dinv); (void)hipFree(L->dref_start); (void)hipFree(L->dcoarse); (void)hipFree(L->dtables);
     for (auto& t : L->htables) { (void)hipFree((void*)t.bucket); (void)hipFree((void*)t.pos); (void)hipFree((void*)((uintptr_t)t.bits & ~(uintptr_t)3)); }
```

Measured after the change: 8474 (median of 6 runs). +1.6%, better.
